# megaease/easevoice-trainer

Hardware: AMD Instinct MI355X
Metric: audio-seconds/sec trained (s2) (higher is better)
Workload: dtype bf16; 1 GPU; s2 SoVITS generator+discriminator GAN step, batch=16/GPU, 4 s 32 kHz clips (T=200 frames), configs/s2.json, random-init weights; global_batch=16, parallelism=dp1, launch=hip-graph replay (3 graphs/step)

## Files before the change

easevoice_trainer_amd/csrc/conv1d.hip:

```cpp
#include "evt_common.h"
#include "../../include/evt.h"
#include "conv_p.h"
#include "wgrad_epi.h"

extern "C" int evt_grouped_supported(const evt_conv1d_params* c);
extern "C" int evt_grouped_fwd(const evt_conv1d_params* c, const void* x, const void* w_reg, const float* bias, void* y,
                               void* stream);
extern "C" int evt_grouped_bwd_data(const evt_conv1d_params* c, const void* dy, const void* y, const void* w_reg,
                                    void* dx, void* stream);
extern "C" int evt_grouped_bwd_data_add(const evt_conv1d_params* c, const void* dy, const void* y, const void* w_reg,
                                        const void* dx_add, void* dx, void* stream);
extern "C" int evt_grouped_bwd_weight(const evt_conv1d_params* c, const void* x, const void* dy, const void* y,
                                      float* dw, void* stream);

extern "C" int evt_small_kind(const evt_conv1d_params* c);
extern "C" int evt_cout1_fwd(const evt_conv1d_params* c, const void* x, const void* w_reg, const float* bias, void* y,
                             void* stream);
extern "C" int evt_cout1_bwd_weight(const evt_conv1d_params* c, const void* x, const void* dy, const void* y, float* dw,
                                    float* dbias, float* ws, long ws_floats, void* stream);
extern "C" int evt_cin1_bwd_weight(const evt_conv1d_params* c, const void* x, const void* dy, const void* y, float* dw,
                                   float* dbias, float* ws, long ws_floats, void* stream);
extern "C" int evt_cin1_fwd(const evt_conv1d_params* c, const void* x, const void* w_reg, const float* bias, void* y,
                            void* stream);
extern "C" int evt_cin1_bwd_data(const evt_conv1d_params* c, const void* dy, const void* y, const void* w_reg,
// ... 1107 lines not shown
  const int d1 = c->transposed ? c->cout : c->cin / c->groups;
  o->d0 = d0; o->d1 = d1; o->k = c->k; o->stride = c->stride;
  pick_ck(c->dtype, d1, c->k, 1, &o->reg_ck, &o->reg_nchunk, &o->reg_kp);
  o->reg_elems = (int64_t)d0 * o->reg_nchunk * o->reg_kp * o->reg_ck;
  if (c->stride == 1) {
    pick_ck(c->dtype, d0, c->k, 1, &o->alt_ck, &o->alt_nchunk, &o->alt_kp);
    o->alt_nphase = 1;
  } else {
    const int J = (c->k + c->stride - 1) / c->stride;
    pick_ck(c->dtype, d0, J, 1, &o->alt_ck, &o->alt_nchunk, &o->alt_kp);
    o->alt_nphase = c->stride;
  }
  o->alt_elems = (int64_t)o->alt_nphase * d1 * o->alt_nchunk * o->alt_kp * o->alt_ck;
  return EVT_OK;
}

int evt_conv1d_fwd(const evt_conv1d_params* c, const void* x, const void* w_reg, const void* w_alt,
                   const float* bias, const void* res, void* y, void* stream) {
  int rc = valid(c);
  if (rc) return rc;
  if (!x || !y) return EVT_EINVAL;
  hipStream_t st = (hipStream_t)stream;
  const bool use_igemm = c->impl != EVT_IMPL_NAIVE && igemm_ok(c);
  if (c->impl == EVT_IMPL_IGEMM && !use_igemm) return EVT_ENOTSUP;
  const int lout = evt_conv1d_lout(c);
  evt_wlayout l; evt_conv1d_layout(c, &l);
  if (w_reg && evt_conv::rows16_eligible(c, c->nseq * c->lin, c->cout, c->cin,
                                         res || c->in_slope != 1.f || c->out_act != EVT_ACT_NONE))
    return evt_conv::launch_rows16(x, w_reg, bias, y, c->nseq * c->lin, c->cout, c->cin, st);
  evt_set_last_tag("conv_naive_fwd");
  if (c->impl != EVT_IMPL_NAIVE && !res && evt_grouped_supported(c)) {
    if (!w_reg) return EVT_EINVAL;
    evt_set_last_tag("grouped_fwd");
    return evt_grouped_fwd(c, x, w_reg, bias, y, stream);
  }
  if (c->impl != EVT_IMPL_NAIVE && !res && evt_small_kind(c) == 1) {
    if (!w_reg) return EVT_EINVAL;
    return evt_cout1_fwd(c, x, w_reg, bias, y, stream);
  }
  if (c->impl != EVT_IMPL_NAIVE && !res && evt_small_kind(c) == 2) {
    if (!w_reg) return EVT_EINVAL;
    return evt_cin1_fwd(c, x, w_reg, bias, y, stream);
  }
  if (!use_igemm) {
    if (!w_reg) return EVT_EINVAL;
    NvP p = make_nvp(c);
    p.x = x; p.w = w_reg; p.bias = bias; p.res = res; p.y = y;
    const long total = (long)c->nseq * lout * c->cout;
    const int blocks = (int)((total + 255) / 256 > 65535 * 8 ? 65535 * 8 : (total + 255) / 256);
    if (c->dtype == EVT_DT_HALF) hipLaunchKernelGGL(conv_naive_fwd<h16_t>, dim3(blocks), dim3(256), 0, st, p);
    else hipLaunchKernelGGL(conv_naive_fwd<float>, dim3(blocks), dim3(256), 0, st, p);
    return evt_check_launch();
  }
  const void* w = c->transposed ? w_alt : w_reg;
  if (!w) return EVT_EINVAL;
  ConvP p{};
  p.x = x; p.xact = nullptr; p.w = w; p.bias = bias; p.res = res; p.gate = nullptr; p.y = y;
  p.nseq = c->nseq; p.Lin = c->lin; p.Lout = lout; p.Cin = c->cin; p.Cout = c->cout;
  p.in_slope = c->in_slope; p.xact_kind = 0; p.xact_slope = 1.f; p.out_act = c->out_act; p.out_slope = c->out_slope;
  p.gate_slope = 1.f;
  int nphase = 1;
  if (!c->transposed) {
    p.KHp = l.reg_kp; p.nchunk = l.reg_nchunk;
    p.s_in = c->stride; p.dil = c->dil; p.off_in = -c->pad;
    p.s_out = 1; p.off_out = 0; p.off_out_phase = 0; p.Q = lout; p.w_phase_stride = 0;
  } else {
    p.KHp = l.alt_kp; p.nchunk = l.alt_nchunk; p.dil = 1; p.s_in = 1;
    if (c->stride == 1) {
      p.off_in = c->pad - (c->k - 1); p.s_out = 1; p.off_out = 0; p.off_out_phase = 0; p.Q = lout;
      p.w_phase_stride = 0;
    } else {
      const int J = (c->k + c->stride - 1) / c->stride;
      nphase = c->stride;
      p.off_in = -(J - 1); p.s_out = c->stride; p.off_out = -c->pad; p.off_out_phase = 1;
      p.Q = (lout - 1 + c->pad) / c->stride + 1;
      p.w_phase_stride = (long)c->cout * l.alt_nchunk * l.alt_kp * l.alt_ck;
    }
  }
  return launch_igemm(c->dtype, p, c->cout, c->cin, nphase, st, c->impl == EVT_IMPL_AUTO);
}

int evt_conv1d_bwd_data(const evt_conv1d_params* c, const void* dy, const void* y, const void* w_reg,
                        const void* w_alt, const void* x, const void* dx_add, void* dx, void* stream) {
  int rc = valid(c);
  if (rc) return rc;
  if (!dy || !dx) return EVT_EINVAL;
  if (c->out_act != EVT_ACT_NONE && !y) return EVT_EINVAL;
  if (c->in_slope != 1.f && !x) return EVT_EINVAL;
  hipStream_t st = (hipStream_t)stream;
  const bool use_igemm = c->impl != EVT_IMPL_NAIVE && igemm_ok(c);
  if (c->impl == EVT_IMPL_IGEMM && !use_igemm) return EVT_ENOTSUP;
  const int lout = evt_conv1d_lout(c);
  evt_wlayout l; evt_conv1d_layout(c, &l);
  const void* ysv = c->out_act != EVT_ACT_NONE ? y : nullptr;
  const void* gate = c->in_slope != 1.f ? x : nullptr;
  if (w_alt && evt_conv::rows16_eligible(c, c->nseq * c->lin, c->cin, c->cout, ysv || gate || dx_add))
    return evt_conv::launch_rows16(dy, w_alt, nullptr, dx, c->nseq * c->lin, c->cin, c->cout, st);
  evt_set_last_tag("conv_naive_bwd_data");
  if (c->impl != EVT_IMPL_NAIVE && !gate && evt_grouped_supported(c)) {
    if (!w_reg) return EVT_EINVAL;
    evt_set_last_tag("grouped_bwd_data");
    return evt_grouped_bwd_data_add(c, dy, y, w_reg, dx_add, dx, stream);
  }
  if (c->impl != EVT_IMPL_NAIVE && evt_small_kind(c) != 0) {
    if (!w_reg) return EVT_EINVAL;
    rc = evt_small_kind(c) == 1 ? evt_cout1_bwd_data(c, dy, y, w_reg, gate, dx_add, dx, stream)
                                : evt_cin1_bwd_data(c, dy, y, w_reg, gate, dx_add, dx, stream);
    if (rc != EVT_ENOTSUP) return rc;
  }
  if (!use_igemm) {
    if (!w_reg) return EVT_EINVAL;
    NvP p = make_nvp(c);
    p.x = dy; p.y_in = ysv; p.w = w_reg; p.gate = gate; p.res = dx_add; p.y = dx;
    const long total = (long)c->nseq * c->lin * c->cin;
    const int blocks = (int)((total + 255) / 256 > 65535 * 8 ? 65535 * 8 : (total + 255) / 256);
    if (c->dtype == EVT_DT_HALF) hipLaunchKernelGGL(conv_naive_bwd_data<h16_t>, dim3(blocks), dim3(256), 0, st, p);
    else hipLaunchKernelGGL(conv_naive_bwd_data<float>, dim3(blocks), dim3(256), 0, st, p);
    return evt_check_launch();
  }
  const void* w = c->transposed ? w_reg : w_alt;
  if (!w) return EVT_EINVAL;
  ConvP p{};
  p.x = dy; p.xact = ysv; p.w = w; p.bias = nullptr; p.res = dx_add; p.gate = gate; p.y = dx;
  p.nseq = c->nseq; p.Lin = lout; p.Lout = c->lin; p.Cin = c->cout; p.Cout = c->cin;
  p.in_slope = 1.f; p.xact_kind = c->out_act; p.xact_slope = c->out_slope; p.out_act = EVT_ACT_NONE;
  p.out_slope = 1.f; p.gate_slope = c->in_slope;
  int nphase = 1;
  if (!c->transposed) {
    p.KHp = l.alt_kp; p.nchunk = l.alt_nchunk;
    if (c->stride == 1) {
      p.s_in = 1; p.dil = c->dil; p.off_in = c->pad - (c->k - 1) * c->dil;
      p.s_out = 1; p.off_out = 0; p.off_out_phase = 0; p.Q = c->lin; p.w_phase_stride = 0;
    } else {
      const int J = (c->k + c->stride - 1) / c->stride;
      nphase = c->stride;
      p.s_in = 1; p.dil = 1; p.off_in = -(J - 1);
      p.s_out = c->stride; p.off_out = -c->pad; p.off_out_phase = 1;
      p.Q = (c->lin - 1 + c->pad) / c->stride + 1;
      p.w_phase_stride = (long)c->cin * l.alt_nchunk * l.alt_kp * l.alt_ck;
    }
  } else {
    p.KHp = l.reg_kp; p.nchunk = l.reg_nchunk;
    p.s_in = c->stride; p.dil = 1; p.off_in = -c->pad;
    p.s_out = 1; p.off_out = 0; p.off_out_phase = 0; p.Q = c->lin; p.w_phase_stride = 0;
  }
  return launch_igemm(c->dtype, p, c->cin, c->cout, nphase, st, c->impl == EVT_IMPL_AUTO);
}

int evt_conv1d_bwd_weight(const evt_conv1d_params* c, const void* x, const void* dy, const void* y, float* dw,
                          float* dbias, void* stream) {
  return evt_conv1d_bwd_weight_parts(c, x, dy, y, dw, dbias, nullptr, stream);
}

int evt_conv1d_bwd_weight_parts(const evt_conv1d_params* c, const void* x, const void* dy, const void* y, float* dw,
                                float* dbias, evt_wgrad_parts* sp, void* stream) {
  int rc = valid(c);
  if (rc) return rc;
  if (!x || !dy || !dw) return EVT_EINVAL;
  int used_host = 0;
  if (sp) {
    sp->used = 0;
    if (sp->parts < 1 || !sp->used_dev || sp->prev_used < 0 || sp->prev_used > sp->parts) return EVT_EINVAL;
    if (sp->parts > 1 && (!sp->dw_extra || sp->part_stride <= 0)) return EVT_EINVAL;
    if (sp->ws && sp->ws_floats <= 0) return EVT_EINVAL;
  }
  if (c->out_act != EVT_ACT_NONE && !y) return EVT_EINVAL;
  hipStream_t st = (hipStream_t)stream;
  const int lout = evt_conv1d_lout(c);
  const void* ysv = c->out_act != EVT_ACT_NONE ? y : nullptr;
  evt_wlayout l; evt_conv1d_layout(c, &l);
  const bool grouped = c->impl != EVT_IMPL_NAIVE && evt_grouped_supported(c);
  const bool igemm_path = !grouped && c->impl != EVT_IMPL_NAIVE && igemm_ok(c) && l.reg_kp <= 64;
  WgP p{};
  p.dw = dw; p.nseq = c->nseq; p.KH = c->k; p.KHp = l.reg_kp; p.s = c->stride; p.dil = c->dil; p.off = -c->pad;
  if (!c->transposed) {
    p.A = dy; p.Aact = ysv; p.aact_kind = c->out_act; p.aact_slope = c->out_slope; p.a_slope = 1.f;
    p.B = x; p.Bact = nullptr; p.bact_kind = 0; p.bact_slope = 1.f; p.b_slope = c->in_slope;
    p.LA = lout; p.CA = c->cout; p.LB = c->lin; p.CB = c->cin; p.Q = lout;
  } else {
    p.A = x; p.Aact = nullptr; p.aact_kind = 0; p.aact_slope = 1.f; p.a_slope = c->in_slope;
    p.B = dy; p.Bact = ysv; p.bact_kind = c->out_act; p.bact_slope = c->out_slope; p.b_slope = 1.f;
    p.LA = c->lin; p.CA = c->cin; p.LB = lout; p.CB = c->cout; p.Q = c->lin;
  }
  p.dbias = nullptr;
  if (sp) {
    p.dw_extra = sp->dw_extra; p.part_stride = sp->part_stride; p.parts = sp->parts; p.prev_used = sp->prev_used;
    p.db_part = sp->db_part; p.used = sp->used_dev; p.used_host = &used_host; p.dirty0 = sp->dirty0 || sp->prev_used > 0;
  }
  const bool gemm_w = igemm_path && c->impl == EVT_IMPL_AUTO && !c->transposed && evt_conv::wgrad_gemm_eligible(p, c->dtype);
  const bool halo_w = !gemm_w && igemm_path && c->impl == EVT_IMPL_AUTO && evt_conv::wgrad_halo_eligible(p, c->dtype);
  const bool deep_w = !gemm_w && !halo_w && igemm_path && c->impl == EVT_IMPL_AUTO && evt_conv::wgrad_deep_eligible(p, c->dtype);
  const bool ring_w = !deep_w && !halo_w && igemm_path && c->impl == EVT_IMPL_AUTO && evt_conv::wgrad_ring_eligible(p, c->dtype);
  const bool cin1 = !grouped && c->impl != EVT_IMPL_NAIVE && evt_small_kind(c) == 2;
  const bool cout1 = !grouped && c->impl != EVT_IMPL_NAIVE && evt_small_kind(c) == 1;
  const bool fuse_bias = dbias && ((igemm_path && c->dtype == EVT_DT_HALF && !c->transposed) || cin1 || cout1);
  float* ws = sp ? sp->ws : nullptr;
  const long ws_floats = sp ? (long)sp->ws_floats : 0;
  if (dbias && !fuse_bias) {
    const long rows = (long)c->nseq * lout;
    const int V = c->dtype == EVT_DT_HALF ? 8 : 4;
    int blocks;
    float* wsb = nullptr;
    if (c->cout % V == 0 && c->cout / V <= 256) {
      long rpb = (rows + 255) / 256;
      if (rpb < 16) rpb = 16;
      blocks = (int)((rows + rpb - 1) / rpb);
      if (ws && blocks >= 2 && (long)blocks * c->cout <= ws_floats) wsb = ws;
      if (c->dtype == EVT_DT_HALF)
        hipLaunchKernelGGL(colsum_act2<h16_t>, dim3(blocks), dim3(256), 0, st, (const h16_t*)dy, (const h16_t*)ysv,
                           dbias, rows, c->cout, c->out_act, c->out_slope, (int)rpb, wsb);
      else
        hipLaunchKernelGGL(colsum_act2<float>, dim3(blocks), dim3(256), 0, st, (const float*)dy, (const float*)ysv,
                           dbias, rows, c->cout, c->out_act, c->out_slope, (int)rpb, wsb);
    } else {
      const int rpb = 64;
      blocks = (int)((rows + rpb - 1) / rpb);
      if (ws && blocks >= 2 && (long)blocks * c->cout <= ws_floats) wsb = ws;
      if (c->dtype == EVT_DT_HALF)
        hipLaunchKernelGGL(colsum_act<h16_t>, dim3(blocks), dim3(256), 0, st, (const h16_t*)dy, (const h16_t*)ysv,
                           dbias, rows, c->cout, c->out_act, c->out_slope, rpb, wsb);
      else
        hipLaunchKernelGGL(colsum_act<float>, dim3(blocks), dim3(256), 0, st, (const float*)dy, (const float*)ysv,
                           dbias, rows, c->cout, c->out_act, c->out_slope, rpb, wsb);
    }
    rc = evt_check_launch();
    if (rc) return rc;
    if (wsb) {
      rc = evt_conv::launch_fold_partials(wsb, c->cout, blocks, dbias, c->cout, st);
      if (rc) return rc;
    }
  }
  evt_set_last_tag("conv_naive_bwd_weight");
  if (grouped) {
    evt_set_last_tag("grouped_bwd_weight");
    return evt_grouped_bwd_weight(c, x, dy, y, dw, stream);
  }
  if (cout1) return evt_cout1_bwd_weight(c, x, dy, y, dw, dbias, ws, ws_floats, stream);
  if (cin1) return evt_cin1_bwd_weight(c, x, dy, y, dw, dbias, ws, ws_floats, stream);
  const bool use_igemm = igemm_path;
  if (c->impl == EVT_IMPL_IGEMM && !use_igemm) return EVT_ENOTSUP;
  if (!use_igemm) {
    NvP p = make_nvp(c);
    p.x = x; p.res = dy; p.y_in = ysv; p.dw = dw;
    const int d1n = c->transposed ? c->cout : c->cin / c->groups;
    const int d0n = c->transposed ? c->cin : c->cout;
    const long elems = (long)d0n * d1n * c->k;
    const long pos = (long)c->nseq * (c->transposed ? c->lin : lout);
    long split = (4096 + elems - 1) / elems;
    const long maxsplit = (pos + 2047) / 2048;
    if (split > maxsplit) split = maxsplit;
    if (split < 1) split = 1;
    p.nsplit = (int)split;
    if (c->dtype == EVT_DT_HALF)
      hipLaunchKernelGGL(conv_naive_bwd_weight<h16_t>, dim3((unsigned)elems, p.nsplit), dim3(256), 0, st, p);
    else
      hipLaunchKernelGGL(conv_naive_bwd_weight<float>, dim3((unsigned)elems, p.nsplit), dim3(256), 0, st, p);
    return evt_check_launch();
  }
  if (gemm_w) {
    p.dbias = fuse_bias ? dbias : nullptr;
    p.parts = 0;
    return evt_conv::launch_wgrad_gemm(p, st);
  }
  if (halo_w || deep_w || ring_w) {
    p.dbias = fuse_bias ? dbias : nullptr;
    if (!p.dbias) p.db_part = nullptr;
    rc = halo_w ? evt_conv::launch_wgrad_halo(p, st) : (deep_w ? evt_conv::launch_wgrad_deep(p, st) : evt_conv::launch_wgrad_ring(p, st));
    if (sp) sp->used = used_host;
    return rc;
  }
  if (c->dtype == EVT_DT_HALF) {
    p.dbias = fuse_bias ? dbias : nullptr;
    p.ws = ws; p.ws_floats = ws_floats;
    if (p.parts < 2) p.parts = 0;
    rc = launch_wgrad_tr(p, st);
    if (sp && rc != EVT_ENOTSUP) sp->used = used_host;
    if (rc != EVT_ENOTSUP) return rc;
    p.parts = 0;
    if (fuse_bias) {
      const long rows = (long)c->nseq * lout;
      hipLaunchKernelGGL(colsum_act<h16_t>, dim3((int)((rows + 63) / 64)), dim3(256), 0, st, (const h16_t*)dy,
                         (const h16_t*)ysv, dbias, rows, c->cout, c->out_act, c->out_slope, 64, (float*)nullptr);
      rc = evt_check_launch();
      if (rc) return rc;
    }
  }
  p.dbias = nullptr;
  return launch_wgrad(c->dtype, p, st);
}

}
```

easevoice_trainer_amd/csrc/conv_deep.hip:

```cpp
#include "conv_p.h"
#include "wgrad_epi.h"

namespace evt_conv {
namespace {

__device__ __attribute__((aligned(256))) unsigned int g_zero_page[64];

typedef __attribute__((address_space(1))) const void* gptr_t;
typedef __attribute__((address_space(3))) void* lptr_t;

__device__ __forceinline__ void glds16(const void* g, void* l) {
  __builtin_amdgcn_global_load_lds((gptr_t)g, (lptr_t)l, 16, 0, 0);
}

constexpr int BM = 128, BN = 128, BK = 64;

template <int TM, int TN, int MI, int NJ>
__device__ __forceinline__ void store_tile_staged(const ConvP& p, unsigned char* smem, const f32x4 (&acc)[MI][NJ], int wr,
                                                  int wc, int n, int g, int yi, int pb, int phase, int total_units) {
  constexpr int PITCH = TM * 2 + 16;
  constexpr int CPR = TM / 8;
  constexpr int RPP = 256 / CPR;
  f32x4 bv[MI];
#pragma unroll
// ... 380 lines not shown
          "=&v"(bh[3]), "=&v"(bh[4])
        : "v"(aa[0]), "v"(aa[1]), "v"(aa[2]), "v"(aa[3]), "v"(ba)
        : "memory");
  } else {
    asm volatile(
        "ds_read_b64_tr_b16 %0, %18 offset:8192\n\t"
        "ds_read_b64_tr_b16 %4, %18 offset:9216\n\t"
        "ds_read_b64_tr_b16 %1, %19 offset:8192\n\t"
        "ds_read_b64_tr_b16 %5, %19 offset:9216\n\t"
        "ds_read_b64_tr_b16 %2, %20 offset:8192\n\t"
        "ds_read_b64_tr_b16 %6, %20 offset:9216\n\t"
        "ds_read_b64_tr_b16 %3, %21 offset:8192\n\t"
        "ds_read_b64_tr_b16 %7, %21 offset:9216\n\t"
        "ds_read_b64_tr_b16 %8, %22 offset:2048\n\t"
        "ds_read_b64_tr_b16 %13, %22 offset:2304\n\t"
        "ds_read_b64_tr_b16 %9, %22 offset:6144\n\t"
        "ds_read_b64_tr_b16 %14, %22 offset:6400\n\t"
        "ds_read_b64_tr_b16 %10, %22 offset:10240\n\t"
        "ds_read_b64_tr_b16 %15, %22 offset:10496\n\t"
        "ds_read_b64_tr_b16 %11, %22 offset:14336\n\t"
        "ds_read_b64_tr_b16 %16, %22 offset:14592\n\t"
        "ds_read_b64_tr_b16 %12, %22 offset:18432\n\t"
        "ds_read_b64_tr_b16 %17, %22 offset:18688\n\t"
        "s_waitcnt lgkmcnt(0)\n\t"
        : "=&v"(al[0]), "=&v"(al[1]), "=&v"(al[2]), "=&v"(al[3]), "=&v"(ah[0]), "=&v"(ah[1]), "=&v"(ah[2]), "=&v"(ah[3]),
          "=&v"(bl[0]), "=&v"(bl[1]), "=&v"(bl[2]), "=&v"(bl[3]), "=&v"(bl[4]), "=&v"(bh[0]), "=&v"(bh[1]), "=&v"(bh[2]),
          "=&v"(bh[3]), "=&v"(bh[4])
        : "v"(aa[0]), "v"(aa[1]), "v"(aa[2]), "v"(aa[3]), "v"(ba)
        : "memory");
  }
  union { uint4 u; h16x8 v; } r;
#pragma unroll
  for (int i = 0; i < 4; ++i) { r.u = make_uint4(al[i].x, al[i].y, ah[i].x, ah[i].y); a[i] = r.v; }
#pragma unroll
  for (int t = 0; t < WKT; ++t) { r.u = make_uint4(bl[t].x, bl[t].y, bh[t].x, bh[t].y); b[t] = r.v; }
}

__global__ __launch_bounds__(256, 2) void wgrad_deep(WgP p, int stages_per_split) {
  extern __shared__ __attribute__((aligned(1024))) unsigned char smem[];
  const int tid = threadIdx.x, lane = tid & 63;
  const int wave = __builtin_amdgcn_readfirstlane(tid >> 6);
  const int j16 = lane & 15, g8 = lane >> 4;
  const int wr = wave >> 1, wc = wave & 1;

  int bx = blockIdx.x;
  int ch, tgi, atile;
  if (p.xcd_order) {
    const int xcd = bx & 7, j = bx >> 3;
    const int na = (p.CA >> 7) >> 1, nc = p.nchunk >> 2;
    const int cl = j % nc, r = j / nc;
    tgi = r % p.ntapgrp;
    const int al = r / p.ntapgrp;
    atile = (xcd & 1) * na + al;
    ch = (xcd >> 1) * nc + cl;
  } else {
    ch = bx % p.nchunk; bx /= p.nchunk;
    tgi = bx % p.ntapgrp;
    atile = bx / p.ntapgrp;
  }
  const int t0 = tgi * WKT;
  const int ntap = min(WKT, p.KHp - t0);
  const int a0 = atile * 128;

  const h16_t* Ag = reinterpret_cast<const h16_t*>(p.A);
  const h16_t* Bg = reinterpret_cast<const h16_t*>(p.B);
  const int total_units = p.nseq * p.Q;
  const int nstages = (total_units + WPOS - 1) / WPOS;
  const int st_begin = blockIdx.y * stages_per_split;
  const int st_end = min(nstages, st_begin + stages_per_split);
  if (st_begin >= st_end) return;

  const h16_t* zsrc = reinterpret_cast<const h16_t*>(g_zero_page);
  int arow[4], acol[4];
#pragma unroll
  for (int i = 0; i < 4; ++i) {
    arow[i] = wave * 16 + i * 4 + (lane >> 4);
    const int f = 2 * ((arow[i] & 3) | (((arow[i] >> 3) & 1) << 2));
    acol[i] = a0 + (((lane & 15) ^ f) * 8);
  }
  const int brow = wave * 16 + (lane >> 2);
  const int bcol = ch * 32 + (((lane & 3) ^ (2 * ((brow >> 3) & 1))) * 8);

  auto issue = [&](int st, int buf) {
    unsigned char* base = smem + buf * WSTAGE;
    const int u0 = st * WPOS;
#pragma unroll
    for (int i = 0; i < 4; ++i) {
      const int u = u0 + arow[i];
      const h16_t* src = u < total_units ? Ag + (long)u * p.CA + acol[i] : zsrc;
      glds16(src, base + wave * 4096 + i * 1024);
    }
    const int u = u0 + brow;
    const bool uok = u < total_units;
    const int seq = uok ? u / p.Q : 0;
    const int q = u - seq * p.Q;
    const int r0 = q * p.s + t0 * p.dil + p.off;
    const h16_t* rsrc = Bg + ((long)seq * p.LB + r0) * p.CB + bcol;
#pragma unroll
    for (int t = 0; t < WKT; ++t) {
      const int r = r0 + t * p.dil;
      const bool ok = uok && (unsigned)r < (unsigned)p.LB;
      const h16_t* src = ok ? rsrc + (long)t * p.dil * p.CB : zsrc;
      glds16(src, base + WA_BYTES + t * WB_BYTES + wave * 1024);
    }
  };

  f32x4 acc[4][WKT];
#pragma unroll
  for (int i = 0; i < 4; ++i)
#pragma unroll
    for (int t = 0; t < WKT; ++t) acc[i][t] = f32x4{0.f, 0.f, 0.f, 0.f};
  const bool do_bias = p.dbias != nullptr && ch == 0 && tgi == 0;
  f32x4 bacc[4];
#pragma unroll
  for (int i = 0; i < 4; ++i) bacc[i] = f32x4{0.f, 0.f, 0.f, 0.f};

  const unsigned lds0 = (unsigned)(uintptr_t)smem;
  const int frow = g8 * 8 + (j16 >> 2);
  const int fa = 2 * ((frow & 3) | (((frow >> 3) & 1) << 2));
  const int fb = 2 * ((frow >> 3) & 1);
  const int half = (j16 & 1) * 8;
  int a_off[4];
#pragma unroll
  for (int i = 0; i < 4; ++i) a_off[i] = frow * 256 + (((wr * 8 + i * 2 + ((j16 & 3) >> 1)) ^ fa) * 16) + half;
  const int b_off = WA_BYTES + frow * 64 + (((wc * 2 + ((j16 & 3) >> 1)) ^ fb) * 16) + half;

  issue(st_begin, 0);
  for (int st = st_begin; st < st_end; ++st) {
    const int buf = (st - st_begin) & 1;
    __syncthreads();
    if (st + 1 < st_end) issue(st + 1, buf ^ 1);
    const unsigned sbase = lds0 + buf * WSTAGE;
    unsigned aa[4];
#pragma unroll
    for (int i = 0; i < 4; ++i) aa[i] = sbase + a_off[i];
    const unsigned ba = sbase + b_off;
    h16x8 a[4], b[WKT];
    tr_load_step<0>(aa, ba, a, b);
#pragma unroll
    for (int t = 0; t < WKT; ++t)
      if (t < ntap)
#pragma unroll
        for (int i = 0; i < 4; ++i) acc[i][t] = EVT_MFMA_16x16x32(a[i], b[t], acc[i][t], 0, 0, 0);
    if (do_bias) wg_bias_mma<4>(bacc, a, wc);
    tr_load_step<1>(aa, ba, a, b);
#pragma unroll
    for (int t = 0; t < WKT; ++t)
      if (t < ntap)
#pragma unroll
        for (int i = 0; i < 4; ++i) acc[i][t] = EVT_MFMA_16x16x32(a[i], b[t], acc[i][t], 0, 0, 0);
    if (do_bias) wg_bias_mma<4>(bacc, a, wc);
  }
  if (do_bias) wg_finish_bias_mma<4>(p, bacc, a0, wr, wc, g8, j16, blockIdx.y);
  wg_finish<4, WKT>(p, smem, acc, ntap, a0, ch, t0, wr, wc, g8, j16, blockIdx.y);
}

constexpr int GKT = 4;
constexpr int GSTAGE = WA_BYTES + GKT * WB_BYTES;

template <int KS>
__device__ __forceinline__ void tr_load_step_g(const unsigned (&aa)[4], unsigned ba, h16x8 (&a)[4], h16x8 (&b)[GKT]) {
  uint2 al[4], ah[4], bl[GKT], bh[GKT];
  if constexpr (KS == 0) {
    asm volatile(
        "ds_read_b64_tr_b16 %0, %16 offset:0\n\t"
        "ds_read_b64_tr_b16 %4, %16 offset:1024\n\t"
        "ds_read_b64_tr_b16 %1, %17 offset:0\n\t"
        "ds_read_b64_tr_b16 %5, %17 offset:1024\n\t"
        "ds_read_b64_tr_b16 %2, %18 offset:0\n\t"
        "ds_read_b64_tr_b16 %6, %18 offset:1024\n\t"
        "ds_read_b64_tr_b16 %3, %19 offset:0\n\t"
        "ds_read_b64_tr_b16 %7, %19 offset:1024\n\t"
        "ds_read_b64_tr_b16 %8, %20 offset:0\n\t"
        "ds_read_b64_tr_b16 %12, %20 offset:256\n\t"
        "ds_read_b64_tr_b16 %9, %20 offset:4096\n\t"
        "ds_read_b64_tr_b16 %13, %20 offset:4352\n\t"
        "ds_read_b64_tr_b16 %10, %20 offset:8192\n\t"
        "ds_read_b64_tr_b16 %14, %20 offset:8448\n\t"
        "ds_read_b64_tr_b16 %11, %20 offset:12288\n\t"
        "ds_read_b64_tr_b16 %15, %20 offset:12544\n\t"
        "s_waitcnt lgkmcnt(0)\n\t"
        : "=&v"(al[0]), "=&v"(al[1]), "=&v"(al[2]), "=&v"(al[3]), "=&v"(ah[0]), "=&v"(ah[1]), "=&v"(ah[2]), "=&v"(ah[3]),
          "=&v"(bl[0]), "=&v"(bl[1]), "=&v"(bl[2]), "=&v"(bl[3]), "=&v"(bh[0]), "=&v"(bh[1]), "=&v"(bh[2]), "=&v"(bh[3])
        : "v"(aa[0]), "v"(aa[1]), "v"(aa[2]), "v"(aa[3]), "v"(ba)
        : "memory");
  } else {
    asm volatile(
        "ds_read_b64_tr_b16 %0, %16 offset:8192\n\t"
        "ds_read_b64_tr_b16 %4, %16 offset:9216\n\t"
        "ds_read_b64_tr_b16 %1, %17 offset:8192\n\t"
        "ds_read_b64_tr_b16 %5, %17 offset:9216\n\t"
        "ds_read_b64_tr_b16 %2, %18 offset:8192\n\t"
        "ds_read_b64_tr_b16 %6, %18 offset:9216\n\t"
        "ds_read_b64_tr_b16 %3, %19 offset:8192\n\t"
        "ds_read_b64_tr_b16 %7, %19 offset:9216\n\t"
        "ds_read_b64_tr_b16 %8, %20 offset:2048\n\t"
        "ds_read_b64_tr_b16 %12, %20 offset:2304\n\t"
        "ds_read_b64_tr_b16 %9, %20 offset:6144\n\t"
        "ds_read_b64_tr_b16 %13, %20 offset:6400\n\t"
        "ds_read_b64_tr_b16 %10, %20 offset:10240\n\t"
        "ds_read_b64_tr_b16 %14, %20 offset:10496\n\t"
        "ds_read_b64_tr_b16 %11, %20 offset:14336\n\t"
        "ds_read_b64_tr_b16 %15, %20 offset:14592\n\t"
        "s_waitcnt lgkmcnt(0)\n\t"
        : "=&v"(al[0]), "=&v"(al[1]), "=&v"(al[2]), "=&v"(al[3]), "=&v"(ah[0]), "=&v"(ah[1]), "=&v"(ah[2]), "=&v"(ah[3]),
          "=&v"(bl[0]), "=&v"(bl[1]), "=&v"(bl[2]), "=&v"(bl[3]), "=&v"(bh[0]), "=&v"(bh[1]), "=&v"(bh[2]), "=&v"(bh[3])
        : "v"(aa[0]), "v"(aa[1]), "v"(aa[2]), "v"(aa[3]), "v"(ba)
        : "memory");
  }
  union { uint4 u; h16x8 v; } r;
#pragma unroll
  for (int i = 0; i < 4; ++i) { r.u = make_uint4(al[i].x, al[i].y, ah[i].x, ah[i].y); a[i] = r.v; }
#pragma unroll
  for (int t = 0; t < GKT; ++t) { r.u = make_uint4(bl[t].x, bl[t].y, bh[t].x, bh[t].y); b[t] = r.v; }
}

template <int NS>
__global__ __launch_bounds__(256, NS > 2 ? 1 : 2) void wgrad_gemm(WgP p, int stages_per_split) {
  extern __shared__ __attribute__((aligned(1024))) unsigned char smem[];
  const int tid = threadIdx.x, lane = tid & 63;
  const int wave = __builtin_amdgcn_readfirstlane(tid >> 6);
  const int j16 = lane & 15, g8 = lane >> 4;
  const int wr = wave >> 1, wc = wave & 1;

  int tile = blockIdx.x, split = blockIdx.y;
  if (p.xcd_order) {
    const int lin = blockIdx.y * gridDim.x + blockIdx.x;
    const int xcd = lin & 7, idx = lin >> 3;
    tile = idx % (int)gridDim.x;
    split = xcd + 8 * (idx / (int)gridDim.x);
  }
  const int ngrp = p.nchunk / GKT;
  const int cg = tile % ngrp;
  const int atile = tile / ngrp;
  const int a0 = atile * 128;

  const h16_t* Ag = reinterpret_cast<const h16_t*>(p.A);
  const h16_t* Bg = reinterpret_cast<const h16_t*>(p.B);
  const int total_units = p.nseq * p.Q;
  const int nstages = (total_units + WPOS - 1) / WPOS;
  const int st_begin = split * stages_per_split;
  const int st_end = min(nstages, st_begin + stages_per_split);
  if (st_begin >= st_end) return;

  const h16_t* zsrc = reinterpret_cast<const h16_t*>(g_zero_page);
  int arow[4], acol[4];
#pragma unroll
  for (int i = 0; i < 4; ++i) {
    arow[i] = wave * 16 + i * 4 + (lane >> 4);
    const int f = 2 * ((arow[i] & 3) | (((arow[i] >> 3) & 1) << 2));
    acol[i] = a0 + (((lane & 15) ^ f) * 8);
  }
  const int brow = wave * 16 + (lane >> 2);
  const int bcol = cg * 128 + (((lane & 3) ^ (2 * ((brow >> 3) & 1))) * 8);

  auto issue = [&](int st, int buf) {
    unsigned char* base = smem + buf * GSTAGE;
    const int u0 = st * WPOS;
#pragma unroll
    for (int i = 0; i < 4; ++i) {
      const int u = u0 + arow[i];
      const h16_t* src = u < total_units ? Ag + (long)u * p.CA + acol[i] : zsrc;
      glds16(src, base + wave * 4096 + i * 1024);
    }
    const int u = u0 + brow;
    const bool uok = u < total_units;
    const h16_t* rsrc = Bg + (long)(uok ? u : 0) * p.CB + bcol;
#pragma unroll
    for (int t = 0; t < GKT; ++t) glds16(uok ? rsrc + t * 32 : zsrc, base + WA_BYTES + t * WB_BYTES + wave * 1024);
  };

  f32x4 acc[4][GKT];
#pragma unroll
  for (int i = 0; i < 4; ++i)
#pragma unroll
    for (int t = 0; t < GKT; ++t) acc[i][t] = f32x4{0.f, 0.f, 0.f, 0.f};
  const int bgrp = ngrp < 4 ? ngrp : 4;
  const bool do_bias = p.dbias != nullptr && cg < bgrp && wc == 0;
  bool mine[4];
#pragma unroll
  for (int i = 0; i < 4; ++i) mine[i] = do_bias && (i % bgrp) == cg;
  h16x8 ones;
#pragma unroll
  for (int e = 0; e < 8; ++e) ones[e] = (evt_hn)1.0f;
  f32x4 bacc[4];
#pragma unroll
  for (int i = 0; i < 4; ++i) bacc[i] = f32x4{0.f, 0.f, 0.f, 0.f};

  const unsigned lds0 = (unsigned)(uintptr_t)smem;
  const int frow = g8 * 8 + (j16 >> 2);
  const int fa = 2 * ((frow & 3) | (((frow >> 3) & 1) << 2));
  const int fb = 2 * ((frow >> 3) & 1);
  const int half = (j16 & 1) * 8;
  int a_off[4];
#pragma unroll
  for (int i = 0; i < 4; ++i) a_off[i] = frow * 256 + (((wr * 8 + i * 2 + ((j16 & 3) >> 1)) ^ fa) * 16) + half;
  const int b_off = WA_BYTES + frow * 64 + (((wc * 2 + ((j16 & 3) >> 1)) ^ fb) * 16) + half;

  const int nst = st_end - st_begin;
  constexpr int G = 4 + GKT;
#pragma unroll
  for (int s = 0; s < NS - 1; ++s)
    if (s < nst) issue(st_begin + s, s);
  for (int st = st_begin; st < st_end; ++st) {
    const int s = st - st_begin;
    const int buf = s % NS;
    wait_groups<G, NS - 2>(min(NS - 2, nst - 1 - s));
// ... 189 lines not shown
        "ds_read_b64_tr_b16 %5, %11 offset:1024\n\t"
        "ds_read_b64_tr_b16 %2, %12 offset:0\n\t"
        "ds_read_b64_tr_b16 %6, %12 offset:1024\n\t"
        "ds_read_b64_tr_b16 %3, %13 offset:0\n\t"
        "ds_read_b64_tr_b16 %7, %13 offset:1024\n\t"
        "ds_read_b64_tr_b16 %8, %14 offset:0\n\t"
        "ds_read_b64_tr_b16 %9, %14 offset:256\n\t"
        "s_waitcnt lgkmcnt(0)\n\t"
        : "=&v"(al[0]), "=&v"(al[1]), "=&v"(al[2]), "=&v"(al[3]), "=&v"(ah[0]), "=&v"(ah[1]), "=&v"(ah[2]), "=&v"(ah[3]), "=&v"(bl[0]), "=&v"(bh[0])
        : "v"(aa[0]), "v"(aa[1]), "v"(aa[2]), "v"(aa[3]), "v"(ba)
        : "memory");
    } else {
    asm volatile(
        "ds_read_b64_tr_b16 %0, %10 offset:8192\n\t"
        "ds_read_b64_tr_b16 %4, %10 offset:9216\n\t"
        "ds_read_b64_tr_b16 %1, %11 offset:8192\n\t"
        "ds_read_b64_tr_b16 %5, %11 offset:9216\n\t"
        "ds_read_b64_tr_b16 %2, %12 offset:8192\n\t"
        "ds_read_b64_tr_b16 %6, %12 offset:9216\n\t"
        "ds_read_b64_tr_b16 %3, %13 offset:8192\n\t"
        "ds_read_b64_tr_b16 %7, %13 offset:9216\n\t"
        "ds_read_b64_tr_b16 %8, %14 offset:2048\n\t"
        "ds_read_b64_tr_b16 %9, %14 offset:2304\n\t"
        "s_waitcnt lgkmcnt(0)\n\t"
        : "=&v"(al[0]), "=&v"(al[1]), "=&v"(al[2]), "=&v"(al[3]), "=&v"(ah[0]), "=&v"(ah[1]), "=&v"(ah[2]), "=&v"(ah[3]), "=&v"(bl[0]), "=&v"(bh[0])
        : "v"(aa[0]), "v"(aa[1]), "v"(aa[2]), "v"(aa[3]), "v"(ba)
        : "memory");
    }
    union { uint4 u; h16x8 v; } r;
#pragma unroll
    for (int i = 0; i < 4; ++i) { r.u = make_uint4(al[i].x, al[i].y, ah[i].x, ah[i].y); a[i] = r.v; }
#pragma unroll
    for (int t = 0; t < 1; ++t) { r.u = make_uint4(bl[t].x, bl[t].y, bh[t].x, bh[t].y); b[t] = r.v; }
  }
};
template <> struct TrStep<4, 3> {
  template <int KS>
  static __device__ __forceinline__ void load(const unsigned (&aa)[4], unsigned ba, h16x8 (&a)[4], h16x8 (&b)[3]) {
    uint2 al[4], ah[4], bl[3], bh[3];
    if constexpr (KS == 0) {
    asm volatile(
        "ds_read_b64_tr_b16 %0, %14 offset:0\n\t"
        "ds_read_b64_tr_b16 %4, %14 offset:1024\n\t"
        "ds_read_b64_tr_b16 %1, %15 offset:0\n\t"
        "ds_read_b64_tr_b16 %5, %15 offset:1024\n\t"
        "ds_read_b64_tr_b16 %2, %16 offset:0\n\t"
        "ds_read_b64_tr_b16 %6, %16 offset:1024\n\t"
        "ds_read_b64_tr_b16 %3, %17 offset:0\n\t"
        "ds_read_b64_tr_b16 %7, %17 offset:1024\n\t"
        "ds_read_b64_tr_b16 %8, %18 offset:0\n\t"
        "ds_read_b64_tr_b16 %11, %18 offset:256\n\t"
        "ds_read_b64_tr_b16 %9, %18 offset:4096\n\t"
        "ds_read_b64_tr_b16 %12, %18 offset:4352\n\t"
        "ds_read_b64_tr_b16 %10, %18 offset:8192\n\t"
        "ds_read_b64_tr_b16 %13, %18 offset:8448\n\t"
        "s_waitcnt lgkmcnt(0)\n\t"
        : "=&v"(al[0]), "=&v"(al[1]), "=&v"(al[2]), "=&v"(al[3]), "=&v"(ah[0]), "=&v"(ah[1]), "=&v"(ah[2]), "=&v"(ah[3]), "=&v"(bl[0]), "=&v"(bl[1]), "=&v"(bl[2]), "=&v"(bh[0]), "=&v"(bh[1]), "=&v"(bh[2])
        : "v"(aa[0]), "v"(aa[1]), "v"(aa[2]), "v"(aa[3]), "v"(ba)
        : "memory");
    } else {
    asm volatile(
        "ds_read_b64_tr_b16 %0, %14 offset:8192\n\t"
        "ds_read_b64_tr_b16 %4, %14 offset:9216\n\t"
        "ds_read_b64_tr_b16 %1, %15 offset:8192\n\t"
        "ds_read_b64_tr_b16 %5, %15 offset:9216\n\t"
        "ds_read_b64_tr_b16 %2, %16 offset:8192\n\t"
        "ds_read_b64_tr_b16 %6, %16 offset:9216\n\t"
        "ds_read_b64_tr_b16 %3, %17 offset:8192\n\t"
        "ds_read_b64_tr_b16 %7, %17 offset:9216\n\t"
        "ds_read_b64_tr_b16 %8, %18 offset:2048\n\t"
        "ds_read_b64_tr_b16 %11, %18 offset:2304\n\t"
        "ds_read_b64_tr_b16 %9, %18 offset:6144\n\t"
        "ds_read_b64_tr_b16 %12, %18 offset:6400\n\t"
        "ds_read_b64_tr_b16 %10, %18 offset:10240\n\t"
        "ds_read_b64_tr_b16 %13, %18 offset:10496\n\t"
        "s_waitcnt lgkmcnt(0)\n\t"
        : "=&v"(al[0]), "=&v"(al[1]), "=&v"(al[2]), "=&v"(al[3]), "=&v"(ah[0]), "=&v"(ah[1]), "=&v"(ah[2]), "=&v"(ah[3]), "=&v"(bl[0]), "=&v"(bl[1]), "=&v"(bl[2]), "=&v"(bh[0]), "=&v"(bh[1]), "=&v"(bh[2])
        : "v"(aa[0]), "v"(aa[1]), "v"(aa[2]), "v"(aa[3]), "v"(ba)
        : "memory");
    }
    union { uint4 u; h16x8 v; } r;
#pragma unroll
    for (int i = 0; i < 4; ++i) { r.u = make_uint4(al[i].x, al[i].y, ah[i].x, ah[i].y); a[i] = r.v; }
#pragma unroll
    for (int t = 0; t < 3; ++t) { r.u = make_uint4(bl[t].x, bl[t].y, bh[t].x, bh[t].y); b[t] = r.v; }
  }
};
template <> struct TrStep<4, 5> {
  template <int KS>
  static __device__ __forceinline__ void load(const unsigned (&aa)[4], unsigned ba, h16x8 (&a)[4], h16x8 (&b)[5]) {
    uint2 al[4], ah[4], bl[5], bh[5];
    if constexpr (KS == 0) {
    asm volatile(
        "ds_read_b64_tr_b16 %0, %18 offset:0\n\t"
        "ds_read_b64_tr_b16 %4, %18 offset:1024\n\t"
        "ds_read_b64_tr_b16 %1, %19 offset:0\n\t"
        "ds_read_b64_tr_b16 %5, %19 offset:1024\n\t"
        "ds_read_b64_tr_b16 %2, %20 offset:0\n\t"
        "ds_read_b64_tr_b16 %6, %20 offset:1024\n\t"
        "ds_read_b64_tr_b16 %3, %21 offset:0\n\t"
        "ds_read_b64_tr_b16 %7, %21 offset:1024\n\t"
        "ds_read_b64_tr_b16 %8, %22 offset:0\n\t"
        "ds_read_b64_tr_b16 %13, %22 offset:256\n\t"
        "ds_read_b64_tr_b16 %9, %22 offset:4096\n\t"
        "ds_read_b64_tr_b16 %14, %22 offset:4352\n\t"
        "ds_read_b64_tr_b16 %10, %22 offset:8192\n\t"
        "ds_read_b64_tr_b16 %15, %22 offset:8448\n\t"
        "ds_read_b64_tr_b16 %11, %22 offset:12288\n\t"
        "ds_read_b64_tr_b16 %16, %22 offset:12544\n\t"
        "ds_read_b64_tr_b16 %12, %22 offset:16384\n\t"
        "ds_read_b64_tr_b16 %17, %22 offset:16640\n\t"
        "s_waitcnt lgkmcnt(0)\n\t"
        : "=&v"(al[0]), "=&v"(al[1]), "=&v"(al[2]), "=&v"(al[3]), "=&v"(ah[0]), "=&v"(ah[1]), "=&v"(ah[2]), "=&v"(ah[3]), "=&v"(bl[0]), "=&v"(bl[1]), "=&v"(bl[2]), "=&v"(bl[3]), "=&v"(bl[4]), "=&v"(bh[0]), "=&v"(bh[1]), "=&v"(bh[2]), "=&v"(bh[3]), "=&v"(bh[4])
        : "v"(aa[0]), "v"(aa[1]), "v"(aa[2]), "v"(aa[3]), "v"(ba)
        : "memory");
    } else {
    asm volatile(
        "ds_read_b64_tr_b16 %0, %18 offset:8192\n\t"
        "ds_read_b64_tr_b16 %4, %18 offset:9216\n\t"
        "ds_read_b64_tr_b16 %1, %19 offset:8192\n\t"
        "ds_read_b64_tr_b16 %5, %19 offset:9216\n\t"
        "ds_read_b64_tr_b16 %2, %20 offset:8192\n\t"
        "ds_read_b64_tr_b16 %6, %20 offset:9216\n\t"
        "ds_read_b64_tr_b16 %3, %21 offset:8192\n\t"
        "ds_read_b64_tr_b16 %7, %21 offset:9216\n\t"
        "ds_read_b64_tr_b16 %8, %22 offset:2048\n\t"
        "ds_read_b64_tr_b16 %13, %22 offset:2304\n\t"
        "ds_read_b64_tr_b16 %9, %22 offset:6144\n\t"
        "ds_read_b64_tr_b16 %14, %22 offset:6400\n\t"
        "ds_read_b64_tr_b16 %10, %22 offset:10240\n\t"
        "ds_read_b64_tr_b16 %15, %22 offset:10496\n\t"
        "ds_read_b64_tr_b16 %11, %22 offset:14336\n\t"
        "ds_read_b64_tr_b16 %16, %22 offset:14592\n\t"
        "ds_read_b64_tr_b16 %12, %22 offset:18432\n\t"
        "ds_read_b64_tr_b16 %17, %22 offset:18688\n\t"
        "s_waitcnt lgkmcnt(0)\n\t"
        : "=&v"(al[0]), "=&v"(al[1]), "=&v"(al[2]), "=&v"(al[3]), "=&v"(ah[0]), "=&v"(ah[1]), "=&v"(ah[2]), "=&v"(ah[3]), "=&v"(bl[0]), "=&v"(bl[1]), "=&v"(bl[2]), "=&v"(bl[3]), "=&v"(bl[4]), "=&v"(bh[0]), "=&v"(bh[1]), "=&v"(bh[2]), "=&v"(bh[3]), "=&v"(bh[4])
        : "v"(aa[0]), "v"(aa[1]), "v"(aa[2]), "v"(aa[3]), "v"(ba)
        : "memory");
    }
    union { uint4 u; h16x8 v; } r;
#pragma unroll
    for (int i = 0; i < 4; ++i) { r.u = make_uint4(al[i].x, al[i].y, ah[i].x, ah[i].y); a[i] = r.v; }
#pragma unroll
    for (int t = 0; t < 5; ++t) { r.u = make_uint4(bl[t].x, bl[t].y, bh[t].x, bh[t].y); b[t] = r.v; }
  }
};

template <int MA> __device__ __forceinline__ int a_swz(int row) {
  return MA == 4 ? 2 * ((row & 3) | (((row >> 3) & 1) << 2)) : 2 * (((row >> 1) & 1) | (((row >> 3) & 1) << 1));
}

template <int MA, int KT, int NS>
__global__ __launch_bounds__(256) void wgrad_ring(WgP p, int stages_per_split) {
  constexpr int AROW = 64 * MA;
  constexpr int ABYTES = WPOS * AROW;
  constexpr int STAGE = ABYTES + KT * WB_BYTES;
  constexpr int G = MA + KT;
  constexpr int RPI = 16 / MA;
  extern __shared__ __attribute__((aligned(1024))) unsigned char smem[];
  const int tid = threadIdx.x, lane = tid & 63;
  const int wave = __builtin_amdgcn_readfirstlane(tid >> 6);
  const int j16 = lane & 15, g8 = lane >> 4;
  const int wr = wave >> 1, wc = wave & 1;

  int bx = blockIdx.x;
  const int split = blockIdx.y;
  const int ch = bx % p.nchunk; bx /= p.nchunk;
  const int tgi = bx % p.ntapgrp;
  const int atile = bx / p.ntapgrp;
  const int t0 = tgi * KT;
  const int ntap = min(KT, p.KHp - t0);
  const int a0 = atile * 32 * MA;

  const h16_t* Ag = reinterpret_cast<const h16_t*>(p.A);
  const h16_t* Bg = reinterpret_cast<const h16_t*>(p.B);
  const int total_units = p.nseq * p.Q;
  const int nstages = (total_units + WPOS - 1) / WPOS;
  const int st_begin = split * stages_per_split;
  const int nst = min(nstages, st_begin + stages_per_split) - st_begin;
  if (nst <= 0) return;

  const h16_t* zsrc = reinterpret_cast<const h16_t*>(g_zero_page);
  int arow[MA], acol[MA];
#pragma unroll
  for (int i = 0; i < MA; ++i) {
    arow[i] = wave * 16 + i * RPI + lane / (4 * MA);
    acol[i] = a0 + (((lane % (4 * MA)) ^ a_swz<MA>(arow[i])) * 8);
  }
  const int brow = wave * 16 + (lane >> 2);
  const int bcol = ch * 32 + (((lane & 3) ^ (2 * ((brow >> 3) & 1))) * 8);

  auto issue = [&](int s) {
    unsigned char* base = smem + (s % NS) * STAGE;
    const int u0 = (st_begin + s) * WPOS;
#pragma unroll
    for (int i = 0; i < MA; ++i) {
      const int u = u0 + arow[i];
      glds16(u < total_units ? Ag + (long)u * p.CA + acol[i] : zsrc, base + wave * (16 * AROW) + i * 1024);
    }
    const int u = u0 + brow;
    const bool uok = u < total_units;
    const int seq = uok ? u / p.Q : 0;
    const int q = u - seq * p.Q;
    const int r0 = q * p.s + t0 * p.dil + p.off;
    const h16_t* rsrc = Bg + ((long)seq * p.LB + r0) * p.CB + bcol;
#pragma unroll
    for (int t = 0; t < KT; ++t) {
      const int r = r0 + t * p.dil;
      const bool ok = uok && (unsigned)r < (unsigned)p.LB;
      glds16(ok ? rsrc + (long)t * p.dil * p.CB : zsrc, base + ABYTES + t * WB_BYTES + wave * 1024);
    }
  };

  f32x4 acc[MA][KT];
#pragma unroll
  for (int i = 0; i < MA; ++i)
#pragma unroll
    for (int t = 0; t < KT; ++t) acc[i][t] = f32x4{0.f, 0.f, 0.f, 0.f};
  const bool do_bias = p.dbias != nullptr && ch == 0 && tgi == 0;
  f32x4 bacc[MA];
#pragma unroll
  for (int i = 0; i < MA; ++i) bacc[i] = f32x4{0.f, 0.f, 0.f, 0.f};

  const unsigned lds0 = (unsigned)(uintptr_t)smem;
  const int frow = g8 * 8 + (j16 >> 2);
  const int fa = a_swz<MA>(frow);
  const int fb = 2 * ((frow >> 3) & 1);
  const int half = (j16 & 1) * 8;
  int a_off[MA];
#pragma unroll
  for (int i = 0; i < MA; ++i) a_off[i] = frow * AROW + (((wr * 2 * MA + i * 2 + ((j16 & 3) >> 1)) ^ fa) * 16) + half;
  const int b_off = ABYTES + frow * 64 + (((wc * 2 + ((j16 & 3) >> 1)) ^ fb) * 16) + half;

#pragma unroll
  for (int s = 0; s < NS - 1; ++s)
    if (s < nst) issue(s);
  for (int s = 0; s < nst; ++s) {
    const int ahead = min(NS - 2, nst - 1 - s);
    wait_groups<G, NS - 2>(ahead);
    __builtin_amdgcn_s_barrier();
    asm volatile("" ::: "memory");
    if (s + NS - 1 < nst) issue(s + NS - 1);
    const unsigned sbase = lds0 + (s % NS) * STAGE;
    unsigned aa[MA];
#pragma unroll
    for (int i = 0; i < MA; ++i) aa[i] = sbase + a_off[i];
    const unsigned ba = sbase + b_off;
    h16x8 a[MA], b[KT];
    TrStep<MA, KT>::template load<0>(aa, ba, a, b);
#pragma unroll
    for (int t = 0; t < KT; ++t)
      if (t < ntap)
#pragma unroll
        for (int i = 0; i < MA; ++i) acc[i][t] = EVT_MFMA_16x16x32(a[i], b[t], acc[i][t], 0, 0, 0);
    if (do_bias) wg_bias_mma<MA>(bacc, a, wc);
    TrStep<MA, KT>::template load<1>(aa, ba, a, b);
#pragma unroll
    for (int t = 0; t < KT; ++t)
      if (t < ntap)
#pragma unroll
        for (int i = 0; i < MA; ++i) acc[i][t] = EVT_MFMA_16x16x32(a[i], b[t], acc[i][t], 0, 0, 0);
    if (do_bias) wg_bias_mma<MA>(bacc, a, wc);
    asm volatile("" ::: "memory");
  }
  if (do_bias) wg_finish_bias_mma<MA>(p, bacc, a0, wr, wc, g8, j16, split);
  wg_finish<MA, KT>(p, smem, acc, ntap, a0, ch, t0, wr, wc, g8, j16, split);
}

}

static int deep_kind(const ConvP& p, int dtype, int out_ch, int k_ch, int nphase);

bool deep_eligible(const ConvP& p, int dtype, int out_ch, int k_ch, int nphase) {
  return deep_kind(p, dtype, out_ch, k_ch, nphase) != 0;
}

static int deep_kind(const ConvP& p, int dtype, int out_ch, int k_ch, int nphase) {
  if (dtype != EVT_DT_HALF) return 0;
  if (k_ch % 32 || out_ch % 64) return 0;
  if (p.xact || p.in_slope != 1.f) return 0;
  if (p.nchunk * 32 != k_ch) return 0;
  if ((long)p.nseq * p.Q >= (1L << 31) - BN) return 0;
  const long units = (long)p.nseq * p.Q;
  constexpr long min128 = 192;
  if (out_ch % BM == 0 && ((units + BN - 1) / BN) * (out_ch / BM) * nphase >= min128) return 2;
  if (k_ch % BK == 0 && ((units + 63) / 64) * (out_ch / 64) * nphase >= 32) return 1;
  return 0;
}


int launch_conv_deep(const ConvP& p_in, int out_ch, int k_ch, int nphase, hipStream_t st) {
  ConvP p = p_in;
  const int kind = deep_kind(p, EVT_DT_HALF, out_ch, k_ch, nphase);
  if (kind == 0) return EVT_ENOTSUP;
  if (kind == 1) {
    p.Y = out_ch / 64;
    p.P = (int)(((long)p.nseq * p.Q + 63) / 64);
    p.U = 0;
    constexpr int NS = 4;
    static bool attr1 = false;
    const size_t lds1 = (size_t)NS * (64 + 64) * 128;
    if (!attr1) {
      if (hipFuncSetAttribute(reinterpret_cast<const void*>(&conv_ring<2, 2, NS>),
                              hipFuncAttributeMaxDynamicSharedMemorySize, (int)lds1) != hipSuccess)
        return EVT_ELAUNCH;
      attr1 = true;
    }
    evt_set_last_tag("conv_ring<bf16, 64, 64, 64, x4>");
    hipLaunchKernelGGL((conv_ring<2, 2, NS>), dim3(8 * ((p.P + 7) / 8) * p.Y, nphase), dim3(256), lds1, st, p);
    return evt_check_launch();
  }
  p.Y = out_ch / BM;
  p.P = (int)(((long)p.nseq * p.Q + BN - 1) / BN);
  p.U = 0;
  const bool short_k = (k_ch / 64) * p.KHp <= 12;
  if (k_ch % 64 || short_k) {
    static bool attr32 = false;
    const size_t lds32 = 2 * STAGE32 > 128 * 272 ? 2 * STAGE32 : 128 * 272;
    if (!attr32) {
      if (hipFuncSetAttribute(reinterpret_cast<const void*>(&conv_deep32), hipFuncAttributeMaxDynamicSharedMemorySize,
                              (int)lds32) != hipSuccess)
        return EVT_ELAUNCH;
      attr32 = true;
    }
    evt_set_last_tag("conv_deep32<bf16, 128, 128, 32>");
    hipLaunchKernelGGL(conv_deep32, dim3(8 * ((p.P + 7) / 8) * p.Y, nphase), dim3(256), lds32, st, p);
    return evt_check_launch();
  }
  static bool attr = false;
  const size_t lds = 2 * STAGE_BYTES;
  if (!attr) {
    if (hipFuncSetAttribute(reinterpret_cast<const void*>(&conv_deep), hipFuncAttributeMaxDynamicSharedMemorySize,
                            (int)lds) != hipSuccess)
      return EVT_ELAUNCH;
    attr = true;
  }
  const int gx = 8 * ((p.P + 7) / 8) * p.Y;
  evt_set_last_tag("conv_deep<bf16, 128, 128, 64>");
  hipLaunchKernelGGL(conv_deep, dim3(gx, nphase), dim3(256), lds, st, p);
  return evt_check_launch();
}

void wgrad_pick_split(const WgP& p, long tiles, int nstages, long target, int min_stages, int* nsplit, int* per) {
  long split = (target + tiles - 1) / tiles;
  if (split > nstages / min_stages) split = nstages / min_stages;
  if (p.parts > 0 && split > p.parts) split = p.parts;
  if (split < 1) split = 1;
  *per = (int)((nstages + split - 1) / split);
  *nsplit = (nstages + *per - 1) / *per;
}

bool wgrad_deep_eligible(const WgP& p, int dtype) {
  if (dtype != EVT_DT_HALF) return false;
  if (p.CA % 128 || p.CB % 32) return false;
  if (p.Aact || p.Bact || p.a_slope != 1.f || p.b_slope != 1.f) return false;
  if (p.LA != p.Q) return false;
  if (p.KHp < 3) return false;
  if ((long)p.nseq * p.Q >= (1L << 31) - WPOS) return false;
  const long tiles = (long)(p.CA / 128) * (p.CB / 32) * ((p.KHp + WKT - 1) / WKT);
  const long nstages = ((long)p.nseq * p.Q + WPOS - 1) / WPOS;
  long split = (1024 + tiles - 1) / tiles;
  if (split > nstages / 8) split = nstages / 8;
  return split >= 1 && tiles * split >= 256;
}

int launch_wgrad_deep(const WgP& p_in, hipStream_t st) {
  WgP p = p_in;
  if (!wgrad_deep_eligible(p, EVT_DT_HALF)) return EVT_ENOTSUP;
  p.nchunk = p.CB / 32;
  p.ntapgrp = (p.KHp + WKT - 1) / WKT;
  const long tiles = (long)(p.CA / 128) * p.nchunk * p.ntapgrp;
  p.xcd_order = ((p.CA / 128) % 2 == 0 && p.nchunk % 4 == 0) ? 1 : 0;
  const int nstages = (int)(((long)p.nseq * p.Q + WPOS - 1) / WPOS);
  int nsplit, per;
  wgrad_pick_split(p, tiles, nstages, p.parts > 0 ? 512 : 1024, 8, &nsplit, &per);
  p.nsplit = nsplit;
  p.now_used = p.prev_used > nsplit ? p.prev_used : nsplit;
  if (p.parts > 0 && p.used_host) *p.used_host = p.now_used;
  static bool attr = false;
  const size_t lds = 2 * WSTAGE;
  if (!attr) {
    if (hipFuncSetAttribute(reinterpret_cast<const void*>(&wgrad_deep), hipFuncAttributeMaxDynamicSharedMemorySize,
                            (int)lds) != hipSuccess)
      return EVT_ELAUNCH;
    attr = true;
  }
  evt_set_last_tag("wgrad_deep<bf16, 128, 5x32, 64>");
  hipLaunchKernelGGL(wgrad_deep, dim3((unsigned)tiles, p.nsplit), dim3(256), lds, st, p, per);
  return evt_check_launch();
}

bool wgrad_gemm_eligible(const WgP& p, int dtype) {
  if (dtype != EVT_DT_HALF) return false;
  if (p.KH != 1 || p.KHp != 1 || p.s != 1 || p.off != 0) return false;
  if (p.CA % 128 || p.CB % 128) return false;
  if (p.Aact || p.Bact || p.a_slope != 1.f || p.b_slope != 1.f) return false;
  if (p.LA != p.Q || p.LB != p.Q) return false;
  const long units = (long)p.nseq * p.Q;
  if (units >= (1L << 31) - WPOS) return false;
  return units >= 2048;
}

static int launch_wgrad_gemm_grid(const WgP& p, long tiles, int per, hipStream_t st);

int launch_wgrad_gemm(const WgP& p_in, hipStream_t st) {
  WgP p = p_in;
  if (!wgrad_gemm_eligible(p, EVT_DT_HALF)) return EVT_ENOTSUP;
  p.nchunk = p.CB / 32;
  p.ntapgrp = 1;
  const long tiles = (long)(p.CA / 128) * (p.CB / 128);
  const int nstages = (int)(((long)p.nseq * p.Q + WPOS - 1) / WPOS);
  constexpr long target = 256;
  long split = (target + tiles - 1) / tiles;
  if (split > nstages / 8) split = nstages / 8;
  if (split < 1) split = 1;
  const int per = (int)((nstages + split - 1) / split);
  split = (nstages + per - 1) / per;
  p.xcd_order = 0;
  if (nstages >= 64) {
    const long s8 = (split + 7) / 8 * 8;
    const int per8 = (int)((nstages + s8 - 1) / s8);
    if ((long)per8 * (s8 - 1) < nstages) {
      split = s8;
      p.xcd_order = 1;
      p.nsplit = (int)split;
      return launch_wgrad_gemm_grid(p, tiles, per8, st);
    }
  }
  p.nsplit = (int)split;
  return launch_wgrad_gemm_grid(p, tiles, per, st);
}

template <int NS>
static int launch_wgrad_gemm_ns(const WgP& p, long tiles, int per, hipStream_t st) {
  static bool attr = false;
  const size_t lds = NS * GSTAGE;
  if (!attr) {
    if (hipFuncSetAttribute(reinterpret_cast<const void*>(&wgrad_gemm<NS>), hipFuncAttributeMaxDynamicSharedMemorySize,
                            (int)lds) != hipSuccess)
      return EVT_ELAUNCH;
    attr = true;
  }
  evt_set_last_tag("wgrad_gemm<bf16, 128, 128, 64, x%d>", NS);
  hipLaunchKernelGGL(wgrad_gemm<NS>, dim3((unsigned)tiles, p.nsplit), dim3(256), lds, st, p, per);
  return evt_check_launch();
}

static int launch_wgrad_gemm_grid(const WgP& p, long tiles, int per, hipStream_t st) {
  return launch_wgrad_gemm_ns<2>(p, tiles, per, st);
}

template <int MA, int KT, int NS>
static int launch_ring_inst(const WgP& p, int per, hipStream_t st) {
  constexpr size_t lds = (size_t)NS * (WPOS * 64 * MA + KT * WB_BYTES);
  static bool attr = false;
  if (!attr) {
    if (hipFuncSetAttribute(reinterpret_cast<const void*>(&wgrad_ring<MA, KT, NS>),
                            hipFuncAttributeMaxDynamicSharedMemorySize, (int)lds) != hipSuccess)
      return EVT_ELAUNCH;
    attr = true;
  }
  const long tiles = (long)(p.CA / (32 * MA)) * p.nchunk * p.ntapgrp;
  evt_set_last_tag("wgrad_ring<bf16, %d, %dx32, 64, x%d>", 32 * MA, KT, NS);
  hipLaunchKernelGGL((wgrad_ring<MA, KT, NS>), dim3((unsigned)tiles, p.nsplit), dim3(256), lds, st, p, per);
  return evt_check_launch();
}

bool wgrad_ring_eligible(const WgP& p, int dtype) {
  if (dtype != EVT_DT_HALF) return false;
  if (p.CA % 64 || p.CB % 32) return false;
  if (p.Aact || p.Bact || p.a_slope != 1.f || p.b_slope != 1.f) return false;
  if (p.LA != p.Q) return false;
  const long units = (long)p.nseq * p.Q;
  if (units >= (1L << 31) - WPOS || units < 512) return false;
  return true;
}

int launch_wgrad_ring(const WgP& p_in, hipStream_t st) {
  WgP p = p_in;
  if (!wgrad_ring_eligible(p, EVT_DT_HALF)) return EVT_ENOTSUP;
  const int KT = p.KHp <= 1 ? 1 : (p.KHp <= 3 ? 3 : 5);
  p.nchunk = p.CB / 32;
  p.ntapgrp = (p.KHp + KT - 1) / KT;
  const int nstages = (int)(((long)p.nseq * p.Q + WPOS - 1) / WPOS);
  const long tiles128 = p.CA % 128 == 0 ? (long)(p.CA / 128) * p.nchunk * p.ntapgrp : 0;
  const int MA = (tiles128 >= 128 || (tiles128 > 0 && tiles128 * (nstages / 4) >= 512)) ? 4 : 2;
  const long tiles = (long)(p.CA / (32 * MA)) * p.nchunk * p.ntapgrp;
  constexpr long target = 256;
  int nsplit, per;
  wgrad_pick_split(p, tiles, nstages, target, 3, &nsplit, &per);
  p.nsplit = nsplit;
  p.now_used = p.prev_used > nsplit ? p.prev_used : nsplit;
  if (p.parts > 0 && p.used_host) *p.used_host = p.now_used;
#define RING(MA_, KT_) (MA_ == 4 && KT_ == 5 ? launch_ring_inst<MA_, KT_, 3>(p, per, st) : launch_ring_inst<MA_, KT_, 4>(p, per, st))
  if (MA == 4) return KT == 1 ? RING(4, 1) : (KT == 3 ? RING(4, 3) : RING(4, 5));
  return KT == 1 ? RING(2, 1) : (KT == 3 ? RING(2, 3) : RING(2, 5));
#undef RING
}

}
```

easevoice_trainer_amd/csrc/conv_p.h:

```cpp
#pragma once
#include "evt_common.h"
#include "../../include/evt.h"
#include <cstdlib>

namespace evt_conv {

struct ConvP {
  const void* x;
  const void* xact;
  const void* w;
  const float* bias;
  const void* res;
  const void* gate;
  void* y;
  int nseq, Lin, Lout, Cin, Cout;
  int KHp;
  int s_in, dil, off_in;
  int s_out, off_out, off_out_phase;
  int Q, U;
  int nchunk;
  long w_phase_stride;
  float in_slope;
  int xact_kind;
  float xact_slope;
  int out_act;
  float out_slope;
  float gate_slope;
  int P, Y;
};

struct WgP {
  const void* A;
  const void* Aact;
  const void* B;
  const void* Bact;
  float* dw;
  int nseq, LA, LB, CA, CB;
  int KH, KHp, s, dil, off, Q;
  int nchunk;
  float a_slope, b_slope;
  int aact_kind, bact_kind;
  float aact_slope, bact_slope;
  int nsplit;
  int ntapgrp;
  int xcd_order;
  float* dbias;
  float* dw_extra;
  long part_stride;
  int parts;
  int prev_used;
  int now_used;
  int dirty0;
  float* db_part;
  int* used;
  int* used_host;
  float* ws;
  long ws_floats;
};

bool deep_eligible(const ConvP& p, int dtype, int out_ch, int k_ch, int nphase);
int launch_conv_deep(const ConvP& p, int out_ch, int k_ch, int nphase, hipStream_t st);
bool narrow_eligible(const ConvP& p, int dtype, int out_ch, int k_ch, int nphase);
int launch_conv_narrow(const ConvP& p, int out_ch, int k_ch, int nphase, hipStream_t st);
bool wgrad_deep_eligible(const WgP& p, int dtype);
int launch_wgrad_deep(const WgP& p, hipStream_t st);
bool wgrad_gemm_eligible(const WgP& p, int dtype);
int launch_wgrad_gemm(const WgP& p, hipStream_t st);
bool wgrad_ring_eligible(const WgP& p, int dtype);
int launch_wgrad_ring(const WgP& p, hipStream_t st);
bool wgrad_halo_eligible(const WgP& p, int dtype);
int launch_wgrad_halo(const WgP& p, hipStream_t st);
int launch_fold_partials(const float* part, long stride, int nb, float* out, long n, hipStream_t st);
int launch_fold_partials2(const float* part, long stride, int nb, float* out, long n, float* out2, long n2, hipStream_t st);
void wgrad_pick_split(const WgP& p, long tiles, int nstages, long target, int min_stages, int* nsplit, int* per);

bool rows16_eligible(const struct evt_conv1d_params* c, int rows, int n_out, int k_red, bool fused);
int launch_rows16(const void* x, const void* w, const float* bias, void* y, int M, int N, int K, hipStream_t st);

}
```

easevoice_trainer_amd/csrc/wgrad_epi.h:

```cpp
#pragma once
#include "conv_p.h"

namespace evt_conv {

__device__ __forceinline__ float* wg_slab(const WgP& p, int s) {
  return s == 0 ? p.dw : p.dw_extra + (long)(s - 1) * p.part_stride;
}

template <int MI, int NT>
__device__ __forceinline__ void wg_store_slab(const WgP& p, float* slab, bool add, float* scratch,
                                              const f32x4 (&acc)[MI][NT], int ntap, int a0, int ch, int t0, int wr, int wc,
                                              int g8, int j16) {
  constexpr int PITCH = NT * 32 + 4;
  constexpr int CPR = NT * 8;
  const int tid = threadIdx.x;
  if constexpr (NT == 1) {
#pragma unroll
    for (int i = 0; i < MI; ++i)
#pragma unroll
      for (int r = 0; r < 4; ++r) {
        const int a = a0 + wr * 16 * MI + i * 16 + g8 * 4 + r;
        float* dst = slab + (((long)a * p.nchunk + ch) * p.KHp + t0) * 32 + wc * 16 + j16;
        *dst = add ? *dst + acc[i][0][r] : acc[i][0][r];
      }
    return;
  }
#pragma unroll
  for (int i = 0; i < MI; ++i) {
    __syncthreads();
#pragma unroll
    for (int t = 0; t < NT; ++t)
#pragma unroll
      for (int r = 0; r < 4; ++r) scratch[(wr * 16 + g8 * 4 + r) * PITCH + t * 32 + wc * 16 + j16] = acc[i][t][r];
    __syncthreads();
    for (int c = tid; c < 32 * CPR; c += 256) {
      const int lr = c / CPR, cc = c - lr * CPR;
      if (cc >= ntap * 8) continue;
      const int a = a0 + (lr >> 4) * 16 * MI + i * 16 + (lr & 15);
      float* dst = slab + (((long)a * p.nchunk + ch) * p.KHp + t0) * 32 + cc * 4;
      f32x4 v = *reinterpret_cast<const f32x4*>(scratch + lr * PITCH + cc * 4);
      if (add) {
        const f32x4 o = *reinterpret_cast<const f32x4*>(dst);
        v += o;
      }
      *reinterpret_cast<f32x4*>(dst) = v;
    }
  }
}

template <int MI, int NT>
__device__ __forceinline__ void wg_finish(const WgP& p, unsigned char* smem, const f32x4 (&acc)[MI][NT], int ntap, int a0,
                                          int ch, int t0, int wr, int wc, int g8, int j16, int split) {
  if (p.parts > 0) {
    if (blockIdx.x == 0 && blockIdx.y == 0 && threadIdx.x == 0) p.used[0] = p.now_used;
    wg_store_slab<MI, NT>(p, wg_slab(p, split), split == 0 ? p.dirty0 != 0 : split < p.prev_used, reinterpret_cast<float*>(smem), acc, ntap,
                          a0, ch, t0, wr, wc, g8, j16);
    return;
  }
#pragma unroll
  for (int t = 0; t < NT; ++t) {
    if (t >= ntap) continue;
#pragma unroll
    for (int i = 0; i < MI; ++i)
#pragma unroll
      for (int r = 0; r < 4; ++r) {
        const int a = a0 + wr * 16 * MI + i * 16 + g8 * 4 + r;
        const long off = (((long)a * p.nchunk + ch) * p.KHp + t0 + t) * 32 + wc * 16 + j16;
        atomicAdd(p.dw + off, acc[i][t][r]);
      }
  }
}

template <int MI>
__device__ __forceinline__ void wg_bias_mma(f32x4 (&bacc)[MI], const h16x8 (&a)[MI], int wc) {
  h16x8 ones;
#pragma unroll
  for (int e = 0; e < 8; ++e) ones[e] = (evt_hn)1.0f;
#pragma unroll
  for (int i = 0; i < MI; ++i)
    if ((i & 1) == wc) bacc[i] = EVT_MFMA_16x16x32(a[i], ones, bacc[i], 0, 0, 0);
}

__device__ __forceinline__ void wg_finish_bias(const WgP& p, int channel, float bsum, int split);

template <int MI>
__device__ __forceinline__ void wg_finish_bias_mma(const WgP& p, const f32x4 (&bacc)[MI], int a0, int wr, int wc, int g8,
                                                   int j16, int split) {
  if (j16 != 0) return;
#pragma unroll
  for (int i = 0; i < MI; ++i)
    if ((i & 1) == wc)
#pragma unroll
      for (int r = 0; r < 4; ++r) wg_finish_bias(p, a0 + wr * 16 * MI + i * 16 + g8 * 4 + r, bacc[i][r], split);
}

__device__ __forceinline__ void wg_finish_bias(const WgP& p, int channel, float bsum, int split) {
  if (p.parts > 0 && p.db_part) {
    float* d = p.db_part + (long)split * p.CA + channel;
    *d = split < p.prev_used ? *d + bsum : bsum;
    if (channel == 0 && split == 0) p.used[1] = p.now_used;
  } else {
    atomicAdd(p.dbias + channel, bsum);
  }
}

}
```

easevoice_trainer_amd/csrc/wgrad_halo.hip:

```cpp
#include "conv_p.h"
#include "wgrad_epi.h"
#include <cstdlib>
#include <type_traits>

namespace evt_conv {
namespace {

__device__ __attribute__((aligned(256))) unsigned int g_zero_page_h[64];

typedef __attribute__((address_space(1))) const void* gptr_t;
typedef __attribute__((address_space(3))) void* lptr_t;

__device__ __forceinline__ void glds16(const void* g, void* l) {
  __builtin_amdgcn_global_load_lds((gptr_t)g, (lptr_t)l, 16, 0, 0);
}

template <int N> __device__ __forceinline__ void wait_vmcnt() { asm volatile("s_waitcnt vmcnt(%0)" ::"n"(N) : "memory"); }
template <int G, int MAXA>
__device__ __forceinline__ void wait_groups(int ahead) {
  if constexpr (MAXA <= 0) { wait_vmcnt<0>(); }
  else {
    if (ahead >= MAXA) wait_vmcnt<(MAXA * G > 63 ? 63 : MAXA * G)>();
    else wait_groups<G, MAXA - 1>(ahead);
  }
// ... 16 lines not shown
template <int MA> __device__ __forceinline__ int a_swz(int row) {
  return MA == 4 ? 2 * ((row & 3) | (((row >> 3) & 1) << 2))
                 : (MA == 2 ? 2 * (((row >> 1) & 1) | (((row >> 3) & 1) << 1)) : 2 * ((row >> 3) & 1));
}

constexpr int HPOS = 64;
constexpr int HROWS = 128;
constexpr int HWIN = HROWS * 64;

template <int MA, int NT, int NS>
__global__ __launch_bounds__(256) void wgrad_halo(WgP p, int spq, int stages_per_split) {
  constexpr int AROW = 64 * MA;
  constexpr int ABYTES = HPOS * AROW;
  constexpr int STAGE = ABYTES + HWIN;
  constexpr int G = MA + 2;
  constexpr int RPI = 16 / MA;
  extern __shared__ __attribute__((aligned(1024))) unsigned char smem[];
  const int tid = threadIdx.x, lane = tid & 63;
  const int wave = __builtin_amdgcn_readfirstlane(tid >> 6);
  const int j16 = lane & 15, g8 = lane >> 4;
  const int wr = wave >> 1, wc = wave & 1;

  const int ch = blockIdx.x % p.nchunk;
  const int a0 = (blockIdx.x / p.nchunk) * 32 * MA;

  const h16_t* Ag = reinterpret_cast<const h16_t*>(p.A);
  const h16_t* Bg = reinterpret_cast<const h16_t*>(p.B);
  const int nstages = p.nseq * spq;
  const int st_begin = blockIdx.y * stages_per_split;
  const int nst = min(nstages, st_begin + stages_per_split) - st_begin;
  if (nst <= 0) return;
  const int hrows = HPOS + (NT - 1) * p.dil;

  const h16_t* zsrc = reinterpret_cast<const h16_t*>(g_zero_page_h);
  int arow[MA], acol[MA];
#pragma unroll
  for (int i = 0; i < MA; ++i) {
    arow[i] = wave * 16 + i * RPI + lane / (4 * MA);
    acol[i] = a0 + (((lane % (4 * MA)) ^ a_swz<MA>(arow[i])) * 8);
  }
  const int brow = wave * 16 + (lane >> 2);
  const int bcol = ch * 32 + (((lane & 3) ^ (2 * ((brow >> 3) & 1))) * 8);

  auto issue = [&](int s) {
    unsigned char* base = smem + (s % NS) * STAGE;
    const int gs = st_begin + s;
    const int seq = gs / spq;
    const int q0 = (gs - seq * spq) * HPOS;
#pragma unroll
    for (int i = 0; i < MA; ++i) {
      const int q = q0 + arow[i];
      glds16(q < p.Q ? Ag + ((long)seq * p.LA + q) * p.CA + acol[i] : zsrc, base + wave * (16 * AROW) + i * 1024);
    }
    const h16_t* rsrc = Bg + ((long)seq * p.LB + q0 + p.off) * p.CB + bcol;
#pragma unroll
    for (int ps = 0; ps < 2; ++ps) {
      const int j = ps * 64 + brow;
      const int r = q0 + p.off + j;
      const bool ok = j < hrows && (unsigned)r < (unsigned)p.LB;
      glds16(ok ? rsrc + (long)j * p.CB : zsrc, base + ABYTES + ps * 4096 + wave * 1024);
    }
  };

  f32x4 acc[MA][NT];
#pragma unroll
  for (int i = 0; i < MA; ++i)
#pragma unroll
    for (int t = 0; t < NT; ++t) acc[i][t] = f32x4{0.f, 0.f, 0.f, 0.f};
  const bool do_bias = p.dbias != nullptr && ch == 0;
  f32x4 bacc[MA];
#pragma unroll
  for (int i = 0; i < MA; ++i) bacc[i] = f32x4{0.f, 0.f, 0.f, 0.f};

  const unsigned lds0 = (unsigned)(uintptr_t)smem;
  const int frow = g8 * 8 + (j16 >> 2);
  const int fa = a_swz<MA>(frow);
  const int half = (j16 & 1) * 8;
  const int cs = (j16 & 3) >> 1;
  int a_off[MA];
#pragma unroll
  for (int i = 0; i < MA; ++i) a_off[i] = frow * AROW + (((wr * 2 * MA + i * 2 + cs) ^ fa) * 16) + half;
  int b_lo[NT], b_hi[NT];
#pragma unroll
  for (int t = 0; t < NT; ++t) {
    const int r0 = frow + t * p.dil, r1 = r0 + 4;
    b_lo[t] = ABYTES + r0 * 64 + (((wc * 2 + cs) ^ (2 * ((r0 >> 3) & 1))) * 16) + half;
    b_hi[t] = ABYTES + r1 * 64 + (((wc * 2 + cs) ^ (2 * ((r1 >> 3) & 1))) * 16) + half;
  }

#pragma unroll
  for (int s = 0; s < NS - 1; ++s)
    if (s < nst) issue(s);
  for (int s = 0; s < nst; ++s) {
    const int ahead = min(NS - 2, nst - 1 - s);
    wait_groups<G, NS - 2>(ahead);
    __builtin_amdgcn_s_barrier();
    asm volatile("" ::: "memory");
    if (s + NS - 1 < nst) issue(s + NS - 1);
    const unsigned sbase = lds0 + (s % NS) * STAGE;
    TrPair fa[2][MA], fb[2][NT];
    auto rd = [&](auto KS, TrPair (&a)[MA], TrPair (&b)[NT]) {
      constexpr int ks = decltype(KS)::value;
#pragma unroll
      for (int i = 0; i < MA; ++i) {
        a[i].lo = tr_rd<ks * 32 * AROW>(sbase + a_off[i]);
        a[i].hi = tr_rd<ks * 32 * AROW + 4 * AROW>(sbase + a_off[i]);
      }
#pragma unroll
      for (int t = 0; t < NT; ++t) {
        b[t].lo = tr_rd<ks * 2048>(sbase + b_lo[t]);
        b[t].hi = tr_rd<ks * 2048>(sbase + b_hi[t]);
      }
    };
    auto landed = [&](TrPair (&a)[MA], TrPair (&b)[NT]) {
#pragma unroll
      for (int i = 0; i < MA; ++i) tr_tie(a[i]);
#pragma unroll
      for (int t = 0; t < NT; ++t) tr_tie(b[t]);
    };
    auto mma = [&](TrPair (&a)[MA], TrPair (&b)[NT]) {
#pragma unroll
      for (int t = 0; t < NT; ++t) {
        const h16x8 bv = tr_join(b[t]);
#pragma unroll
        for (int i = 0; i < MA; ++i) acc[i][t] = EVT_MFMA_16x16x32(tr_join(a[i]), bv, acc[i][t], 0, 0, 0);
      }
      if (do_bias) {
        h16x8 af[MA];
#pragma unroll
        for (int i = 0; i < MA; ++i) af[i] = tr_join(a[i]);
        wg_bias_mma<MA>(bacc, af, wc);
      }
    };
    constexpr bool PIPE = MA * NT * 4 + 2 * (MA + NT) * 4 <= 200;
    rd(std::integral_constant<int, 0>{}, fa[0], fb[0]);
    asm volatile("s_waitcnt lgkmcnt(0)");
    landed(fa[0], fb[0]);
    if constexpr (PIPE) {
      rd(std::integral_constant<int, 1>{}, fa[1], fb[1]);
      mma(fa[0], fb[0]);
      asm volatile("s_waitcnt lgkmcnt(0)");
      landed(fa[1], fb[1]);
      mma(fa[1], fb[1]);
    } else {
      mma(fa[0], fb[0]);
      rd(std::integral_constant<int, 1>{}, fa[0], fb[0]);
      asm volatile("s_waitcnt lgkmcnt(0)");
      landed(fa[0], fb[0]);
      mma(fa[0], fb[0]);
    }
    asm volatile("" ::: "memory");
  }
  if (do_bias) wg_finish_bias_mma<MA>(p, bacc, a0, wr, wc, g8, j16, blockIdx.y);
  wg_finish<MA, NT>(p, smem, acc, NT, a0, ch, 0, wr, wc, g8, j16, blockIdx.y);
}

template <int MA, int NT, int NS>
int launch_inst(const WgP& p, int spq, int per, hipStream_t st) {
  constexpr size_t lds = (size_t)NS * (HPOS * 64 * MA + HWIN);
  static_assert(lds >= 32 * (NT * 32 + 4) * 4, "epilogue scratch");
  static bool attr = false;
  if (!attr) {
    if (hipFuncSetAttribute(reinterpret_cast<const void*>(&wgrad_halo<MA, NT, NS>),
                            hipFuncAttributeMaxDynamicSharedMemorySize, (int)lds) != hipSuccess)
      return EVT_ELAUNCH;
    attr = true;
  }
  const long tiles = (long)(p.CA / (32 * MA)) * p.nchunk;
  evt_set_last_tag("wgrad_halo<bf16, %d, %dx32, 64, x%d>", 32 * MA, NT, NS);
  hipLaunchKernelGGL((wgrad_halo<MA, NT, NS>), dim3((unsigned)tiles, p.nsplit), dim3(256), lds, st, p, spq, per);
  return evt_check_launch();
}

}

bool wgrad_halo_eligible(const WgP& p, int dtype) {
  if (dtype != EVT_DT_HALF) return false;
  if (p.s != 1 || p.KHp != p.KH) return false;
  if (p.KH != 3 && p.KH != 5 && p.KH != 7 && p.KH != 11) return false;
  if ((p.CA % 64 && p.CA != 32) || p.CB % 32) return false;
  if (p.Aact || p.Bact || p.a_slope != 1.f || p.b_slope != 1.f) return false;
  if (p.LA != p.Q) return false;
  if (HPOS + (p.KH - 1) * p.dil > HROWS) return false;
  static const bool all = getenv("EVT_HALO_ALL") != nullptr;
  if (!all && p.CA != 64 && p.CA != 32) return false;
  if (p.CA % 128 == 0 && (long)(p.CA / 128) * (p.CB / 32) >= 128) return false;
  const int spq = (p.Q + HPOS - 1) / HPOS;
  if ((long)spq * HPOS * 10 > (long)p.Q * 13) return false;
  if ((long)p.nseq * spq < 8) return false;
  return true;
}

int launch_wgrad_halo(const WgP& p_in, hipStream_t st) {
  WgP p = p_in;
  if (!wgrad_halo_eligible(p, EVT_DT_HALF)) return EVT_ENOTSUP;
  p.nchunk = p.CB / 32;
  p.ntapgrp = 1;
  const int spq = (p.Q + HPOS - 1) / HPOS;
  const int nstages = p.nseq * spq;
  const long tiles128 = p.CA % 128 == 0 ? (long)(p.CA / 128) * p.nchunk : 0;
  int MA = tiles128 >= 64 ? 4 : 2;
  if (p.CA == 32) MA = 1;
  const long tiles = (long)(p.CA / (32 * MA)) * p.nchunk;
  constexpr long target = 256;
  int nsplit, per;
  wgrad_pick_split(p, tiles, nstages, target, 3, &nsplit, &per);
  p.nsplit = nsplit;
  p.now_used = p.prev_used > nsplit ? p.prev_used : nsplit;
  if (p.parts > 0 && p.used_host) *p.used_host = p.now_used;
#define HALO(MA_, NS_)                                                                                   \
  (p.KH == 3 ? launch_inst<MA_, 3, NS_>(p, spq, per, st)                                                 \
             : p.KH == 5 ? launch_inst<MA_, 5, NS_>(p, spq, per, st)                                     \
                         : p.KH == 7 ? launch_inst<MA_, 7, NS_>(p, spq, per, st) : launch_inst<MA_, 11, NS_>(p, spq, per, st))
  return MA == 4 ? HALO(4, 3) : (MA == 2 ? HALO(2, 4) : HALO(1, 4));
#undef HALO
}

}
```

easevoice_trainer_amd/hip/conv.py:

```python
import ctypes as C
import os
import math

import torch
from torch import nn

from . import lib as L


class ConvSlot:

    __slots__ = ("module", "layout", "reg", "alt", "dw", "bank", "_pcache", "packed_member", "parts", "dw_extra",
                 "db_part", "used", "wg_used", "wg_dirty", "_wgp")

    def __init__(self, module, layout, bank):
        self.module, self.layout, self.bank = module, layout, bank
        self.reg = self.alt = self.dw = None
        self._pcache = {}
        self.packed_member = False
        self.parts, self.dw_extra, self.db_part, self.used, self.wg_used, self._wgp = 1, None, None, None, 0, None
        self.wg_dirty = False

    def params(self, nseq, lin, in_slope, out_act, out_slope):
        key = (nseq, lin, in_slope, out_act, out_slope, self.bank.impl)
# ... 154 lines not shown
            ex_n += (s.parts - 1) * ((s.layout.reg_elems + ALIGN - 1) // ALIGN * ALIGN)
            db_n += s.parts * ((s.layout.d0 + 31) // 32 * 32)
        self._ws = {}
        self.dw_extra_arena = torch.zeros(max(ex_n, 1), dtype=torch.float32, device=device) if self.parts_on else None
        self.db_part_arena = torch.zeros(max(db_n, 1), dtype=torch.float32, device=device) if self.parts_on else None
        for i, (s, (ro, ao)) in enumerate(zip(self.slots, offs)):
            s.reg = self.reg_arena[ro: ro + s.layout.reg_elems]
            s.alt = self.alt_arena[ao: ao + s.layout.alt_elems]
            s.dw = self.dw_arena[ro: ro + s.layout.reg_elems]
            s.used = self.used_all[2 * i: 2 * i + 2]
            if self.parts_on:
                eo, do = ex_offs[i]
                stride = (s.layout.reg_elems + ALIGN - 1) // ALIGN * ALIGN
                s.dw_extra = self.dw_extra_arena[eo: eo + (s.parts - 1) * stride]
                s.db_part = self.db_part_arena[do: do + s.parts * s.layout.d0]
        self._items = self._rows = None
        self._nrows = 0
        self._frags, self._frag_items, self._frag_rows, self._frag_tables = {}, [], [], {}
        self._frag_retired = []

    def build_tables(self):
        items, rows, groups = [], [], []
        self._slot_rows = []
        self._group_of_row = {}
        for i, s in enumerate(self.slots):
            m = s.module
            self._slot_rows.append((len(rows), len(rows) + s.layout.d0))
            v = m.v
            if v.grad is None:
                v.grad = torch.zeros_like(v)
            g = m.weight_g if m.weight_norm else None
            if g is not None and g.grad is None:
                g.grad = torch.zeros_like(g)
            it = L.WPrepItem()
            it.v = v.data_ptr()
            it.g = g.data_ptr() if g is not None else None
            it.reg, it.alt, it.dw = s.reg.data_ptr(), s.alt.data_ptr(), (None if s.packed_member else s.dw.data_ptr())
            it.dv = v.grad.data_ptr()
            it.dg = g.grad.data_ptr() if g is not None else None
            it.lay = s.layout
            it.dtype = self.dt
            it.src_d1 = int(getattr(m, "src_d1", 0))
            if self.parts_on and not s.packed_member:
                it.dw_extra = s.dw_extra.data_ptr() if s.parts > 1 else None
                it.dw_part_stride = (s.layout.reg_elems + 127) // 128 * 128
                it.used = s.used.data_ptr()
                bias = getattr(m, "bias", None)
                if bias is not None and not m.transposed:
                    if bias.grad is None:
                        bias.grad = torch.zeros_like(bias)
                    it.db_part, it.db = s.db_part.data_ptr(), bias.grad.data_ptr()
            items.append(it)
            self._group_of_row[len(rows)] = len(groups)
            rows.extend((i, r) for r in range(s.layout.d0))
            groups.extend((i, r, min(8, s.layout.d0 - r)) for r in range(0, s.layout.d0, 8))
        self._group_of_row[len(rows)] = len(groups)
        self._items = L.struct_to_device(items, self.device)
        self._rows = torch.tensor(rows, dtype=torch.int32, device=self.device).contiguous()
        self._groups = torch.tensor(groups, dtype=torch.int32, device=self.device).contiguous()
        self._nrows = len(rows)
        self._grad_stamp = self._grad_ptrs()

    def _grad_ptrs(self):
        out = []
        for s in self.slots:
            m = s.module
            g = m.weight_g if m.weight_norm else None
            b = getattr(m, "bias", None)
            out.append((m.v.grad.data_ptr() if m.v.grad is not None else 0,
                        g.grad.data_ptr() if (g is not None and g.grad is not None) else 0,
                        b.grad.data_ptr() if (b is not None and b.grad is not None) else 0))
        return out

    def fold(self, lo=None, hi=None):
        if self._items is None:
            self.build_tables()
        lo = 0 if lo is None else lo
        hi = self._nrows if hi is None else hi
        if hi <= lo:
            return
        glo, ghi = self._group_of_row.get(lo), self._group_of_row.get(hi)
        if glo is not None and ghi is not None and os.environ.get("EVT_FOLD_GROUPS", "1") != "0":
            grp = C.c_void_p(self._groups.data_ptr() + 12 * glo)
            L.check(L.lib().evt_wn_fold_groups(L.ptr(self._items), grp, ghi - glo, L.stream_ptr()), "evt_wn_fold_groups")
        else:
            rows = C.c_void_p(self._rows.data_ptr() + 8 * lo)
            L.check(L.lib().evt_wn_fold_multi(L.ptr(self._items), rows, hi - lo, L.stream_ptr()), "evt_wn_fold_multi")
        self._repack_frags(lo, hi)

    def frag(self, slot, which):
        key = (id(slot), which)
        f = self._frags.get(key)
        if f is None:
            lay = slot.layout
            if which == "reg":
                rows, ktot, src, elems = lay.d0, lay.reg_nchunk * lay.reg_kp * lay.reg_ck, slot.reg, lay.reg_elems
            else:
                rows, ktot, src, elems = lay.d1, lay.alt_nchunk * lay.alt_kp * lay.alt_ck, slot.alt, lay.alt_elems
            if elems != rows * ktot or rows % 16 or ktot % 32 or not L.is_half(self.dtype):
                raise L.EvtError(f"no fragment-order form for this image ({which}, {rows} x {ktot}, {self.dtype})")
            if self._items is None:
                self.build_tables()
            f = torch.empty(elems, dtype=self.dtype, device=self.device)
            it = L.FragItem()
            it.src, it.dst, it.rows, it.ktot = src.data_ptr(), f.data_ptr(), rows, ktot
            self._frags[key] = f
            self._frag_items.append(it)
            self._frag_rows.append(self._slot_rows[self.slots.index(slot)])
            self._frag_retired.extend(t for t, _n in self._frag_tables.values() if t is not None)
            self._frag_tables.clear()
            one = L.struct_to_device([it], self.device)
            self._frag_tables[("one", len(self._frag_items))] = (one, 1)
            L.check(L.lib().evt_frag_pack(L.ptr(one), 1, L.stream_ptr()), "evt_frag_pack")
            if not torch.cuda.is_current_stream_capturing():
                items = list(self._frag_items)
                self._frag_tables[(0, self._nrows)] = (L.struct_to_device(items, self.device), len(items))
        return f

    def _repack_frags(self, lo, hi):
        if not self._frag_items:
            return
        tab = self._frag_tables.get((lo, hi))
        if tab is None:
            items = [it for it, (r0, r1) in zip(self._frag_items, self._frag_rows) if r0 < hi and r1 > lo]
            tab = self._frag_tables[(lo, hi)] = (L.struct_to_device(items, self.device) if items else None, len(items))
        if tab[1]:
            L.check(L.lib().evt_frag_pack(L.ptr(tab[0]), tab[1], L.stream_ptr()), "evt_frag_pack")

    def zero_dw(self):
        if self._deferred or self._held:
            self._deferred.clear()
            self._deferred_on.clear()
            self._deferred_bytes = 0
            if self._side is not None:
                torch.cuda.current_stream(self.device).wait_stream(self._side)
            self._held.clear()
        self.dw_arena.zero_()
        self._tables_checked = False
        for s in self.slots:
            s.wg_used, s.wg_dirty = 0, False

    def scratch(self):
        key = torch.cuda.current_stream(self.device).cuda_stream
        ws = self._ws.get(key)
        if ws is None:
            ws = self._ws[key] = torch.empty(4 << 20, dtype=torch.float32, device=self.device)
        return ws

    def side_stream(self):
        if self._side is None:
            self._side = L.role_stream(self.device, "bank")
        return self._side

    def flush_deferred(self):
        if not self._deferred:
            return
        side = self.side_stream()
        side.wait_stream(torch.cuda.current_stream(self.device))
        for st in self._deferred_on:
            side.wait_stream(st)
        self._deferred_on.clear()
        with torch.cuda.stream(side):
            for args in self._deferred:
                _bwd_weight_now(*args)
        self._held.extend((a[1], a[2], a[3]) for a in self._deferred)
        self._deferred.clear()
        self._deferred_bytes = 0

    def join_side(self):
        self.flush_deferred()
        if self._side is not None and self._held:
            torch.cuda.current_stream(self.device).wait_stream(self._side)
        self._held.clear()

    def rows_of(self, modules):
        idx = sorted(i for i, s in enumerate(self.slots) if any(s.module is m for m in modules))
        if not idx or idx != list(range(idx[0], idx[-1] + 1)):
            raise L.EvtError("rows_of: the modules must be a contiguous, non-empty run of this bank's convolutions")
        if self._items is None:
            self.build_tables()
        return self._slot_rows[idx[0]][0], self._slot_rows[idx[-1]][1]

    def check_tables(self):
        if self._items is None:
            self.build_tables()
        elif not getattr(self, "_tables_checked", False) and not torch.cuda.is_current_stream_capturing():
            if self._grad_stamp != self._grad_ptrs():
                self.build_tables()
            self._tables_checked = True

    def grads(self, lo=None, hi=None, join=True):
        if join:
            self.join_side()
        self.check_tables()
        lo = 0 if lo is None else lo
        hi = self._nrows if hi is None else hi
        if hi <= lo:
            return
        rows = C.c_void_p(self._rows.data_ptr() + 8 * lo)
        L.check(L.lib().evt_wn_grad_multi(L.ptr(self._items), rows, hi - lo, L.stream_ptr()), "evt_wn_grad_multi")


class FrozenConv:
    weight_norm, kdims, transposed, groups, dil = False, 1, False, 1, 1

    def __init__(self, weight_fn, bias_fn, cin, cout, k=1, stride=1, padding=0):
        self.weight_fn, self.bias_fn = weight_fn, bias_fn
        self.cin, self.cout, self.k, self.stride, self.pad = cin, cout, k, stride, padding
        self._slot = None

    @property
    def v(self):
        w = self.weight_fn()
        return w if w.dim() == 3 else w.unsqueeze(-1)

    @property
    def bias(self):
        return self.bias_fn() if self.bias_fn is not None else None

    def lout(self, lin):
        return (lin + 2 * self.pad - (self.k - 1) - 1) // self.stride + 1


class FrozenBank:
    weight_grads = False

    def __init__(self, convs, device, impl=L.IMPL_AUTO):
        self.dt, self.dtype, self.device, self.impl = L.DT_F32, torch.float32, torch.device(device), impl
        self.slots, offs, reg_n, alt_n = [], [], 0, 0
        for m in convs:
            lay = conv_layout(self.dt, m.cin, m.cout, m.k, m.stride, m.pad, m.dil, m.groups, m.transposed)
            s = ConvSlot(m, lay, self)
            m._slot = s
            self.slots.append(s)
            offs.append((reg_n, alt_n))
            reg_n += (lay.reg_elems + 127) // 128 * 128
            alt_n += (lay.alt_elems + 127) // 128 * 128
        self.reg_arena = torch.zeros(max(reg_n, 1), dtype=torch.float32, device=device)
        self.alt_arena = torch.zeros(max(alt_n, 1), dtype=torch.float32, device=device)
        for s, (ro, ao) in zip(self.slots, offs):
            s.reg = self.reg_arena[ro: ro + s.layout.reg_elems]
            s.alt = self.alt_arena[ao: ao + s.layout.alt_elems]
        self._stamp = self._items = None

    def prepare(self):
        vs = [s.module.v for s in self.slots]
        stamp = tuple((v.data_ptr(), v._version) for v in vs)
        if stamp == self._stamp:
            return
        items, rows = [], []
        for i, (s, v) in enumerate(zip(self.slots, vs)):
            if v.dtype != torch.float32 or not v.is_contiguous() or v.device != self.device:
                raise L.EvtError("FrozenBank: contiguous fp32 weights on the bank's device expected")
            it = L.WPrepItem()
            it.v, it.g, it.reg, it.alt = v.data_ptr(), None, s.reg.data_ptr(), s.alt.data_ptr()
            it.dw = it.dv = it.dg = None
            it.lay, it.dtype = s.layout, self.dt
            items.append(it)
            rows.extend((i, r) for r in range(s.layout.d0))
        self._items = L.struct_to_device(items, self.device)
        self._rows = torch.tensor(rows, dtype=torch.int32, device=self.device).contiguous()
        L.check(L.lib().evt_wn_fold_multi(L.ptr(self._items), L.ptr(self._rows), len(rows), L.stream_ptr()),
                "evt_wn_fold_multi")
        self._stamp = stamp


PLAIN_X = os.environ.get("EVT_CONV_PLAIN_X", "1") != "0"
TRACE = None


TRACE_RANGES = False


def set_trace(rec, ranges=False):
    global TRACE, TRACE_RANGES
    TRACE = rec
    TRACE_RANGES = bool(ranges) and rec is not None
    L.lib().evt_debug_kernel_tags(1 if rec is not None else 0)


def _t0():
    if TRACE is None:
        return None
    rf = None
    if TRACE_RANGES:
        rf = torch.profiler.record_function(f"evt#{len(TRACE)}")
        rf.__enter__()
    e = torch.cuda.Event(enable_timing=True)
    e.record()
    return e, rf


def _t1(e0, kind, m, nseq, lin, extra_elems):
    e0, rf = e0
    e1 = torch.cuda.Event(enable_timing=True)
    e1.record()
    if rf is not None:
        rf.__exit__(None, None, None)
    lq = lin if m.transposed else m.lout(lin)
    macs = nseq * lq * m.cin * m.cout * m.k // m.groups
    sz = 2 if L.is_half(m._slot.bank.dtype) else 4
    act = nseq * (lin * m.cin + m.lout(lin) * m.cout) + extra_elems
    wbytes = m.v.numel() * (4 if kind == "bwd_weight" else sz)
    shape = (f"{'T' if m.transposed else ''}{m.cin}>{m.cout} k{m.k} s{m.stride} d{m.dil} g{m.groups} "
             f"n{nseq} L{lin}")
    TRACE.append((L.lib().evt_last_kernel_tag().decode(), kind, 2 * macs, act * sz + wbytes, e0, e1, shape, m))


def _t1_elt(e0, name, nbytes, owner):
    e0, rf = e0
    e1 = torch.cuda.Event(enable_timing=True)
    e1.record()
    if rf is not None:
        rf.__exit__(None, None, None)
    TRACE.append((name, "elt", 0, nbytes, e0, e1, name, owner))


def _fwd(slot, x, res, in_slope, out_act, out_slope, out=None):
    m = slot.module
    if x.dim() != 3 or x.size(2) != m.cin or x.dtype != slot.bank.dtype or not x.is_contiguous():
        raise L.EvtError(f"conv input must be contiguous [nseq, L, {m.cin}] {slot.bank.dtype}, got "
                         f"{tuple(x.shape)} {x.dtype} contiguous={x.is_contiguous()}")
    nseq, lin = x.size(0), x.size(1)
    y = out if out is not None else torch.empty((nseq, m.lout(lin), m.cout), dtype=x.dtype, device=x.device)
    if y.shape != (nseq, m.lout(lin), m.cout) or y.dtype != x.dtype or not y.is_contiguous():
        raise L.EvtError("conv output buffer must be contiguous [nseq, Lout, Cout] in the compute dtype")
    if res is not None and (res.shape != y.shape or not res.is_contiguous() or res.dtype != x.dtype):
        raise L.EvtError("residual must match the output")
    p = slot.params(nseq, lin, in_slope, out_act, out_slope)
    bias = m.bias
    e0 = _t0()
    L.check(L.lib().evt_conv1d_fwd(C.byref(p), L.ptr(x), L.ptr(slot.reg), L.ptr(slot.alt),
                                   L.ptr(bias.data if bias is not None else None), L.ptr(res), L.ptr(y),
                                   L.stream_ptr()), "evt_conv1d_fwd")
    if e0 is not None:
        _t1(e0, "fwd", m, nseq, lin, y.numel() if res is not None else 0)
    return y


def _bwd_data(slot, dy, y, x, dx_add, nseq, lin, in_slope, out_act, out_slope):
    m = slot.module
    dx = torch.empty((nseq, lin, m.cin), dtype=dy.dtype, device=dy.device)
    p = slot.params(nseq, lin, in_slope, out_act, out_slope)
    e0 = _t0()
    L.check(L.lib().evt_conv1d_bwd_data(C.byref(p), L.ptr(dy), L.ptr(y if out_act != L.ACT_NONE else None),
                                        L.ptr(slot.reg), L.ptr(slot.alt), L.ptr(x if in_slope != 1.0 else None),
                                        L.ptr(dx_add), L.ptr(dx), L.stream_ptr()), "evt_conv1d_bwd_data")
    if e0 is not None:
        extra = (dy.numel() if out_act != L.ACT_NONE else 0) + (dx.numel() if in_slope != 1.0 else 0) + \
                (dx.numel() if dx_add is not None else 0)
        _t1(e0, "bwd_data", m, nseq, lin, extra)
    return dx


def _bwd_weight(slot, x, dy, y, nseq, lin, in_slope, out_act, out_slope):
    bank = slot.bank
    if slot.packed_member:
        raise L.EvtError("weight gradient of a packed projection member requested on its own: inside a bf16 runtime the "
                         "q / k / v projections of a windowed attention layer run (and are differentiated) as one pack")
    if bank.defer_n > 0 and TRACE is None:
        bank._deferred.append((slot, x, dy, y, nseq, lin, in_slope, out_act, out_slope))
        bank._deferred_on.add(torch.cuda.current_stream(bank.device))
        bank._deferred_bytes += x.numel() * x.element_size() + dy.numel() * dy.element_size()
        if len(bank._deferred) >= bank.defer_n or bank._deferred_bytes >= bank.defer_bytes:
            bank.flush_deferred()
        return
    _bwd_weight_now(slot, x, dy, y, nseq, lin, in_slope, out_act, out_slope)


def _bwd_weight_now(slot, x, dy, y, nseq, lin, in_slope, out_act, out_slope):
    m = slot.module
    p = slot.params(nseq, lin, in_slope, out_act, out_slope)
    dbias = None
    if m.bias is not None:
        if m.bias.grad is None:
            m.bias.grad = torch.zeros_like(m.bias)
        dbias = m.bias.grad
    e0 = _t0()
    if slot.bank.parts_on:
        sp = slot._wgp
        if sp is None:
            sp = slot._wgp = L.WgradParts()
            sp.dw_extra = slot.dw_extra.data_ptr() if slot.parts > 1 else None
            sp.part_stride = (slot.layout.reg_elems + 127) // 128 * 128
            sp.db_part = slot.db_part.data_ptr() if (dbias is not None and not m.transposed) else None
            sp.used_dev = slot.used.data_ptr()
            sp.parts = slot.parts
        sp.prev_used, sp.dirty0 = slot.wg_used, int(slot.wg_dirty)
        ws = slot.bank.scratch()
        sp.ws, sp.ws_floats = ws.data_ptr(), ws.numel()
        L.check(L.lib().evt_conv1d_bwd_weight_parts(C.byref(p), L.ptr(x), L.ptr(dy),
                                                    L.ptr(y if out_act != L.ACT_NONE else None), L.ptr(slot.dw),
                                                    L.ptr(dbias), C.byref(sp), L.stream_ptr()),
                "evt_conv1d_bwd_weight_parts")
        slot.wg_used, slot.wg_dirty = max(slot.wg_used, int(sp.used)), True
    else:
        L.check(L.lib().evt_conv1d_bwd_weight(C.byref(p), L.ptr(x), L.ptr(dy),
                                              L.ptr(y if out_act != L.ACT_NONE else None), L.ptr(slot.dw), L.ptr(dbias),
                                              L.stream_ptr()), "evt_conv1d_bwd_weight")
    if e0 is not None:
        _t1(e0, "bwd_weight", m, nseq, lin, dy.numel() if out_act != L.ACT_NONE else 0)


class ConvFn(torch.autograd.Function):

    @staticmethod
    def forward(ctx, x, anchor, res, slot, in_slope, out_act, out_slope):
        ctx.pre = False
        if in_slope != 1.0 and x.is_cuda and x.dim() == 3 and PLAIN_X and L.lib().evt_conv1d_wants_plain_x(
                C.byref(slot.params(x.size(0), x.size(1), in_slope, out_act, out_slope))):
            xa = torch.empty_like(x)
            e0 = _t0()
            L.check(L.lib().evt_leaky_relu(L.dt_of(x), L.ptr(x), C.c_float(in_slope), L.ptr(xa), C.c_int64(x.numel()),
                                           L.stream_ptr()), "evt_leaky_relu")
            if e0 is not None:
                _t1_elt(e0, "lrelu_kernel", 2 * x.numel() * x.element_size(), slot.module)
            y = _fwd(slot, xa, res, 1.0, out_act, out_slope)
            x, ctx.pre = xa, True
        else:
            y = _fwd(slot, x, res, in_slope, out_act, out_slope)
        ctx.slot, ctx.cfg = slot, (in_slope, out_act, out_slope)
        ctx.has_res = res is not None
        ctx.save_for_backward(x, y if out_act != L.ACT_NONE else None)
        return y

    @staticmethod
    def backward(ctx, dy):
        x, y = ctx.saved_tensors
        slot = ctx.slot
        in_slope, out_act, out_slope = ctx.cfg
        dy = dy.contiguous()
        nseq, lin = x.size(0), x.size(1)
        if out_act != L.ACT_NONE and L.lib().evt_conv1d_wants_plain_dy(
                C.byref(slot.params(nseq, lin, in_slope, out_act, out_slope))):
            dy_eff = torch.empty_like(dy)
            e0 = _t0()
            L.check(L.lib().evt_dact_mul(L.dt_of(dy), L.ptr(dy), L.ptr(y), int(out_act), C.c_float(out_slope),
                                         L.ptr(dy_eff), C.c_int64(dy.numel()), L.stream_ptr()), "evt_dact_mul")
            if e0 is not None:
                _t1_elt(e0, "dact_mul_kernel", 3 * dy.numel() * dy.element_size(), slot.module)
            dy, y, out_act, out_slope = dy_eff, None, L.ACT_NONE, 1.0
        if slot.bank.weight_grads:
            _bwd_weight(slot, x, dy, y, nseq, lin, 1.0 if ctx.pre else in_slope, out_act, out_slope)
        dx = None
        if ctx.needs_input_grad[0]:
            dx = _bwd_data(slot, dy, y, x, None, nseq, lin, in_slope, out_act, out_slope)
        dres = dy if (ctx.has_res and ctx.needs_input_grad[2]) else None
        if dres is not None and out_act != L.ACT_NONE:
            raise L.EvtError("residual + output activation: residual is added after the activation, "
                             "its gradient is dy (supported), but was not expected here")
        return dx, None, dres, None, None, None, None


def _resunit_params(s1, s2, x, slope):
    m1, m2 = s1.module, s2.module
    if (not L.is_half(x.dtype) or not x.is_cuda or not x.is_contiguous() or x.dim() != 3 or m1.cin != m1.cout
            or m2.cin != m2.cout or m1.cin != m2.cin or m1.k != m2.k or m2.dil != 1 or m1.stride != 1 or m2.stride != 1
            or m1.groups != 1 or m2.groups != 1 or m1.transposed or m2.transposed
            or m1.pad != m1.dil * (m1.k - 1) // 2 or m2.pad != (m2.k - 1) // 2 or s1.bank.impl != L.IMPL_AUTO):
        return None
    p = L.ResUnitParams(L.dt_code(x.dtype), x.size(0), x.size(1), m1.cin, m1.k, m1.dil, float(slope))
    return p if L.lib().evt_resunit_supported(C.byref(p)) else None


def _resunit_wide_params(s1, s2, x, slope):
    m1, m2 = s1.module, s2.module
    if (not L.is_half(x.dtype) or not x.is_cuda or not x.is_contiguous() or x.dim() != 3 or m1.cin != m1.cout
            or m2.cin != m2.cout or m1.cin != m2.cin or m1.k != m2.k or m2.dil != 1 or m1.stride != 1 or m2.stride != 1
            or m1.groups != 1 or m2.groups != 1 or m1.transposed or m2.transposed
            or m1.pad != m1.dil * (m1.k - 1) // 2 or m2.pad != (m2.k - 1) // 2 or s1.bank.impl != L.IMPL_AUTO):
        return None
    p = L.ResUnitParams(L.dt_code(x.dtype), x.size(0), x.size(1), m1.cin, m1.k, m1.dil, float(slope))
    return p if L.lib().evt_resunit_wide_supported(C.byref(p)) else None


def _t1_unit(e0, m1, m2, x):
    e0, rf = e0
    e1 = torch.cuda.Event(enable_timing=True)
    e1.record()
    if rf is not None:
        rf.__exit__(None, None, None)
    n, ln, c = x.shape
    macs = n * ln * c * c * (m1.k + m2.k)
    TRACE.append((L.lib().evt_last_kernel_tag().decode(), "fwd", 2 * macs, 4 * x.numel() * 2 + (m1.v.numel() + m2.v.numel()) * 2,
                  e0, e1, f"unit {c}>{c} k{m1.k} d{m1.dil} n{n} L{ln}", m1))


def _lrelu(x, slope, owner=None):
    out = torch.empty_like(x)
    e0 = _t0()
    L.check(L.lib().evt_leaky_relu(L.dt_of(x), L.ptr(x), C.c_float(slope), L.ptr(out), C.c_int64(x.numel()),
                                   L.stream_ptr()), "evt_leaky_relu")
    if e0 is not None:
        _t1_elt(e0, "lrelu_kernel", 2 * x.numel() * x.element_size(), owner)
    return out


def _add3(a, b, c, scale, out, owner):
    e0 = _t0()
    L.check(L.lib().evt_add3_scale(L.dt_of(a), L.ptr(a), L.ptr(b), L.ptr(c), C.c_float(scale), L.ptr(out),
                                   C.c_int64(a.numel()), L.stream_ptr()), "evt_add3_scale")
    if e0 is not None:
        _t1_elt(e0, "add3_scale_kernel", (2 + (b is not None) + (c is not None)) * a.numel() * a.element_size(), owner)
    return out


class ResUnitFn(torch.autograd.Function):

    @staticmethod
    def forward(ctx, x, anchor, s1, s2, slope):
        fused = _resunit_params(s1, s2, x, slope)
        if fused is not None:
            m1, m2 = s1.module, s2.module
            xa, mid_a, y = torch.empty_like(x), torch.empty_like(x), torch.empty_like(x)
            e0 = _t0()
            L.check(L.lib().evt_resunit_fwd(C.byref(fused), L.ptr(x), L.ptr(s1.reg), L.ptr(s2.reg),
                                            L.ptr(m1.bias.data if m1.bias is not None else None),
                                            L.ptr(m2.bias.data if m2.bias is not None else None), L.ptr(xa), L.ptr(mid_a),
                                            L.ptr(y), L.stream_ptr()), "evt_resunit_fwd")
            if e0 is not None:
                _t1_unit(e0, m1, m2, x)
            ctx.s1, ctx.s2, ctx.slope = s1, s2, slope
            ctx.save_for_backward(xa, mid_a)
            return y
        wide = _resunit_wide_params(s1, s2, x, slope)
        if wide is not None:
            m1, m2 = s1.module, s2.module
            xa, mid_a, y = torch.empty_like(x), torch.empty_like(x), torch.empty_like(x)
            e0 = _t0()
            L.check(L.lib().evt_resunit_wide_fwd(C.byref(wide), L.ptr(x), L.ptr(s1.reg), L.ptr(s2.reg),
                                                 L.ptr(m1.bias.data if m1.bias is not None else None),
                                                 L.ptr(m2.bias.data if m2.bias is not None else None), L.ptr(xa),
                                                 L.ptr(mid_a), L.ptr(y), L.stream_ptr()), "evt_resunit_wide_fwd")
            if e0 is not None:
                _t1_unit(e0, m1, m2, x)
            ctx.s1, ctx.s2, ctx.slope = s1, s2, slope
            ctx.save_for_backward(xa, mid_a)
            return y
        xa = _lrelu(x, slope, s1.module)
        mid_a = _fwd(s1, xa, None, 1.0, L.ACT_LRELU, slope)
        y = _fwd(s2, mid_a, x, 1.0, L.ACT_NONE, 1.0)
        ctx.s1, ctx.s2, ctx.slope = s1, s2, slope
        ctx.save_for_backward(xa, mid_a)
# ... 382 lines not shown
```

easevoice_trainer_amd/hip/lib.py:

```python
import ctypes as C
import os

import torch

_HERE = os.path.dirname(os.path.abspath(__file__))
LIB_PATH = os.path.join(os.path.dirname(_HERE), "libevt_hip.so")
LIB_PATH_F16 = os.path.join(os.path.dirname(_HERE), "libevt_hip_f16.so")

DT_F32, DT_BF16, DT_F16 = 0, 1, 2
HALF_DTYPES = (torch.bfloat16, torch.float16)
ACT_NONE, ACT_LRELU, ACT_TANH = 0, 1, 2
IMPL_AUTO, IMPL_NAIVE, IMPL_IGEMM = 0, 1, 2


class EvtError(RuntimeError):
    pass


EVT_OK, EVT_ELAUNCH, EVT_EINVAL, EVT_ENOTSUP = 0, 5, 22, 95


class ConvParams(C.Structure):
    _fields_ = [
        ("dtype", C.c_int32), ("nseq", C.c_int32), ("lin", C.c_int32), ("cin", C.c_int32), ("cout", C.c_int32),
        ("k", C.c_int32), ("stride", C.c_int32), ("pad", C.c_int32), ("dil", C.c_int32), ("groups", C.c_int32),
        ("transposed", C.c_int32), ("in_slope", C.c_float), ("out_act", C.c_int32), ("out_slope", C.c_float),
        ("impl", C.c_int32),
    ]


class ResUnitParams(C.Structure):
    _fields_ = [("dtype", C.c_int32), ("nseq", C.c_int32), ("L", C.c_int32), ("C", C.c_int32), ("k", C.c_int32),
                ("dil", C.c_int32), ("slope", C.c_float)]


class ResUnitFwdJob(C.Structure):
    _fields_ = [("p", ResUnitParams), ("x", C.c_void_p), ("w1_reg", C.c_void_p), ("w2_reg", C.c_void_p),
                ("b1", C.c_void_p), ("b2", C.c_void_p), ("xa", C.c_void_p), ("mid_a", C.c_void_p), ("y", C.c_void_p)]


class ResUnitBwdJob(C.Structure):
    _fields_ = [("p", ResUnitParams), ("dy_scale", C.c_float), ("dy", C.c_void_p), ("xa", C.c_void_p),
                ("mid_a", C.c_void_p), ("w1_alt", C.c_void_p), ("w2_alt", C.c_void_p), ("dx", C.c_void_p),
                ("dmid", C.c_void_p), ("dw1", C.c_void_p), ("dw2", C.c_void_p), ("db1", C.c_void_p), ("db2", C.c_void_p)]


class WLayout(C.Structure):
    _fields_ = [
        ("d0", C.c_int32), ("d1", C.c_int32), ("k", C.c_int32), ("stride", C.c_int32),
        ("reg_ck", C.c_int32), ("reg_nchunk", C.c_int32), ("reg_kp", C.c_int32),
        ("alt_ck", C.c_int32), ("alt_nchunk", C.c_int32), ("alt_kp", C.c_int32), ("alt_nphase", C.c_int32),
        ("reg_elems", C.c_int64), ("alt_elems", C.c_int64),
    ]


class WPrepItem(C.Structure):
    _fields_ = [
        ("v", C.c_void_p), ("g", C.c_void_p), ("reg", C.c_void_p), ("alt", C.c_void_p),
        ("dw", C.c_void_p), ("dv", C.c_void_p), ("dg", C.c_void_p),
        ("lay", WLayout), ("dtype", C.c_int32), ("src_d1", C.c_int32),
        ("dw_extra", C.c_void_p), ("dw_part_stride", C.c_int64), ("db_part", C.c_void_p), ("db", C.c_void_p),
        ("used", C.c_void_p),
    ]


class FragItem(C.Structure):
    _fields_ = [("src", C.c_void_p), ("dst", C.c_void_p), ("rows", C.c_int32), ("ktot", C.c_int32)]


class WgradParts(C.Structure):
    _fields_ = [("dw_extra", C.c_void_p), ("part_stride", C.c_int64), ("db_part", C.c_void_p), ("used_dev", C.c_void_p),
                ("parts", C.c_int32), ("prev_used", C.c_int32), ("used", C.c_int32), ("dirty0", C.c_int32),
                ("ws", C.c_void_p), ("ws_floats", C.c_int64)]


class Seg(C.Structure):
    _fields_ = [("a", C.c_void_p), ("b", C.c_void_p), ("da", C.c_void_p), ("n", C.c_int64),
                ("scale", C.c_float), ("pad_", C.c_int32)]


class KlParams(C.Structure):
    _fields_ = [("B", C.c_int32), ("T", C.c_int32), ("C", C.c_int32), ("time_inner", C.c_int32),
                ("dt_z_p", C.c_int32), ("dt_logs_q", C.c_int32), ("dt_m_p", C.c_int32), ("dt_logs_p", C.c_int32)]


class AdamWSeg(C.Structure):
    _fields_ = [("begin", C.c_int64), ("end", C.c_int64), ("lr", C.c_float), ("weight_decay", C.c_float)]


class AttnParams(C.Structure):
    _fields_ = [
        ("dtype", C.c_int32), ("B", C.c_int32), ("L", C.c_int32), ("H", C.c_int32), ("D", C.c_int32),
        ("x_len", C.c_int32),
        ("q_stride_b", C.c_int64), ("q_stride_l", C.c_int64), ("q_stride_h", C.c_int64),
        ("o_stride_b", C.c_int64), ("o_stride_l", C.c_int64), ("o_stride_h", C.c_int64),
        ("dropout_p", C.c_float), ("seed", C.c_uint32),
    ]


class SampleParams(C.Structure):
    _fields_ = [("V", C.c_int32), ("eos", C.c_int32), ("top_k", C.c_int32), ("no_eos_steps", C.c_int32),
                ("ymax", C.c_int32), ("top_p", C.c_float), ("temperature", C.c_float),
                ("repetition_penalty", C.c_float), ("seed", C.c_uint32), ("noise_rows", C.c_int32)]


class RowSample(C.Structure):
    _fields_ = [("top_k", C.c_int32), ("top_p", C.c_float), ("temperature", C.c_float),
                ("repetition_penalty", C.c_float)]


DEC_POS, DEC_IDX, DEC_YCOUNT, DEC_YLEN, DEC_SEED = 0, 1, 2, 3, 4


class SAChunk(C.Structure):
    _fields_ = [("begin", C.c_int64), ("end", C.c_int64), ("tensor", C.c_int32), ("pad_", C.c_int32)]


class ScaledAdamHP(C.Structure):
    _fields_ = [("lr", C.c_float), ("beta1", C.c_float), ("beta2", C.c_float), ("eps", C.c_float),
                ("scalar_lr_scale", C.c_float), ("scalar_max", C.c_float), ("step", C.c_int32), ("pad_", C.c_int32)]


class MhaParams(C.Structure):
    _fields_ = [("dtype", C.c_int32), ("B", C.c_int32), ("H", C.c_int32), ("D", C.c_int32), ("Tq", C.c_int32),
                ("Tk", C.c_int32), ("window", C.c_int32), ("n_heads_rel", C.c_int32), ("ldq", C.c_int64),
                ("ldk", C.c_int64), ("ldo", C.c_int64), ("scale", C.c_float), ("dropout_p", C.c_float),
                ("site", C.c_uint32), ("pad_", C.c_uint32), ("seed_dev", C.c_void_p)]


_libs = {}
_half = torch.bfloat16


def set_half(dtype) -> None:
    global _half
    if dtype in HALF_DTYPES:
        _half = dtype


def half():
    return _half


def is_half(dtype) -> bool:
    return dtype in HALF_DTYPES


def dt_code(dtype) -> int:
    if dtype == torch.float32:
        return DT_F32
    if dtype in HALF_DTYPES:
        if dtype != _half:
            raise EvtError(f"{dtype} data while the {_half} build of the library is selected: call hip.lib.set_half({dtype}) "
                           "(the engines do, at the top of a step)")
        return DT_BF16 if dtype == torch.bfloat16 else DT_F16
    raise EvtError(f"unsupported dtype {dtype}")


def _check_fresh(handle, LIB_PATH=LIB_PATH):
    csrc = os.path.join(os.path.dirname(_HERE), "csrc")
    if os.environ.get("EVT_ALLOW_STALE_LIB") == "1" or not os.path.isdir(csrc):
        return
    from ..build import source_hash

    have = handle.evt_version().decode()
    want = source_hash()
    if f"src={want}" not in have:
        raise EvtError(f"{LIB_PATH} is stale: built from sources {have.split('src=')[-1]!r}, the tree has {want!r}; "
                       "rebuild with `python -m easevoice_trainer_amd.build` (EVT_ALLOW_STALE_LIB=1 overrides)")


def lib():
    _lib = _libs.get(_half)
    if _lib is None:
        path = LIB_PATH if _half == torch.bfloat16 else LIB_PATH_F16
        if not os.path.exists(path):
            raise EvtError(
                f"{path} not found: build it with `python -m easevoice_trainer_amd.build` "
                "(or __graft_entry__.build()). There is no fallback path.")
        _lib = C.CDLL(path)
        _lib.evt_version.restype = C.c_char_p
        _check_fresh(_lib, path)
        _lib.evt_half_dtype.restype = C.c_int32
        if _lib.evt_half_dtype() != (DT_BF16 if _half == torch.bfloat16 else DT_F16):
            raise EvtError(f"{path} serves half code {_lib.evt_half_dtype()}: not the {_half} build")
        _libs[_half] = _lib
        _lib.evt_conv1d_lout.restype = C.c_int32
        _lib.evt_mel_workspace_floats.restype = C.c_int64
        _lib.evt_workspace_bytes.restype = C.c_int64
        _lib.evt_last_kernel_tag.restype = C.c_char_p
        _lib.evt_resunit_bwd_ws_floats.restype = C.c_int64
        _lib.evt_debug_kernel_tags.restype = None
        for name in ("evt_resunit_fwd_multi_lens", "evt_resunit_wide_fwd_lens", "evt_mask_tail", "evt_resample_rows",
                     "evt_resample_pack_rows", "evt_hubert_front_rows", "evt_clip_rescale_rows", "evt_phone_expand_rows",
                     "evt_bert_embed_ln_rows", "evt_ref_spec_rows", "evt_mish_rows_fwd", "evt_glu_res_rows_fwd",
                     "evt_mean_rows"):
            getattr(_lib, name).restype = C.c_int
        _lib.evt_hubert_front_ws_floats.restype = C.c_int64
    return _lib


def check(rc: int, what: str) -> None:
    if rc != 0:
        raise EvtError(f"{what} failed with code {rc}")


def dt_of(t: torch.Tensor) -> int:
    return dt_code(t.dtype)


def torch_dtype(dt: int) -> torch.dtype:
    return {DT_F32: torch.float32, DT_BF16: torch.bfloat16, DT_F16: torch.float16}[dt]


def ptr(t):
    if t is None:
        return C.c_void_p(0)
    if not t.is_contiguous():
        raise EvtError("non-contiguous tensor passed to the C ABI")
    return C.c_void_p(t.data_ptr())


_hip_rt = None
_role_pools = {}


# ... 62 lines not shown
```

easevoice_trainer_amd/hip/wn.py:

```python
import ctypes as C

import torch

from . import conv as HC
from . import lib as L


class WNStackFn(torch.autograd.Function):
    @staticmethod
    def forward(ctx, x, g_lbh, lens, anchor, in_slots, rs_slots, hidden):
        n_layers, H = len(in_slots), hidden
        B, T, _ = x.shape
        if not x.is_contiguous() or x.size(2) != H or (g_lbh is not None and not g_lbh.is_contiguous()):
            raise L.EvtError("WN stack: contiguous [B, T, H] input and [n_layers, B, 2H] conditioning expected")
        dt = L.dt_of(x)
        rows = B * T
        saved = []
        out = None
        fused = FUSED_FORWARD and _layer_fused(dt, H, in_slots, rs_slots)
        frag_in, frag_rs = _frag_images(in_slots, rs_slots) if fused else (None, None)
        for i in range(n_layers):
            last = i == n_layers - 1
            if fused:
                mi, mr = in_slots[i].module, rs_slots[i].module
                x_in = torch.empty((B, T, 2 * H), dtype=x.dtype, device=x.device)
                acts = torch.empty((B, T, H), dtype=x.dtype, device=x.device)
                acc_out = torch.empty((B, T, H), dtype=x.dtype, device=x.device)
                x_out = None if last else torch.empty_like(acc_out)
                e0 = HC._t0()
                L.check(L.lib().evt_wn_layer_fwd(dt, L.ptr(x), L.ptr(frag_in[i]),
                                                 L.ptr(mi.bias.data if mi.bias is not None else None), L.ptr(frag_rs[i]),
                                                 L.ptr(mr.bias.data if mr.bias is not None else None),
                                                 L.ptr(g_lbh[i] if g_lbh is not None else None), L.ptr(out), L.ptr(lens),
                                                 L.ptr(x_in), L.ptr(acts), L.ptr(x_out), L.ptr(acc_out), B, T, H, mi.k,
                                                 int(last), L.stream_ptr()), "evt_wn_layer_fwd")
                if e0 is not None:
                    _t1_layer(e0, mi, mr, x)
                saved += [x, x_in, acts]
                x, out = x_out, acc_out
                continue
            x_in = HC._fwd(in_slots[i], x, None, 1.0, L.ACT_NONE, 1.0)
            acts = torch.empty((B, T, H), dtype=x.dtype, device=x.device)
            L.check(L.lib().evt_gated_act_fwd(dt, L.ptr(x_in), L.ptr(g_lbh[i] if g_lbh is not None else None), L.ptr(acts),
                                              B, T, H, L.stream_ptr()), "evt_gated_act_fwd")
            rs = HC._fwd(rs_slots[i], acts, None, 1.0, L.ACT_NONE, 1.0)
            acc_out = torch.empty((B, T, H), dtype=x.dtype, device=x.device)
            x_out = None if last else torch.empty_like(acc_out)
            L.check(L.lib().evt_wn_residual_fwd(dt, L.ptr(None if last else x), L.ptr(rs), L.ptr(out), L.ptr(lens), T,
                                                L.ptr(x_out), L.ptr(acc_out), C.c_int64(rows), H, int(last),
                                                L.stream_ptr()), "evt_wn_residual_fwd")
            saved += [x, x_in, acts]
            x, out = x_out, acc_out
        ctx.save_for_backward(lens, g_lbh, *saved)
        ctx.cfg = (in_slots, rs_slots, H, B, T)
        return out

    @staticmethod
    def backward(ctx, dout):
        lens, g_lbh, *saved = ctx.saved_tensors
        in_slots, rs_slots, H, B, T = ctx.cfg
        n_layers = len(in_slots)
        dtype, dev = dout.dtype, dout.device
        dt = L.dt_code(dtype)
        rows = B * T
        dacc = dout.contiguous()
        dx_next = None
        dg32 = torch.zeros((n_layers, B, 2 * H), dtype=torch.float32, device=dev) if g_lbh is not None else None
        fused = FUSED_BACKWARD and _layer_fused(dt, H, in_slots, rs_slots)
        for i in reversed(range(n_layers)):
            last = i == n_layers - 1
            x, x_in, acts = saved[3 * i: 3 * i + 3]
            rs_w = H if last else 2 * H
            if fused:
                si, sr = in_slots[i], rs_slots[i]
                drs = torch.empty((B, T, rs_w), dtype=dtype, device=dev)
                dx_in = torch.empty((B, T, 2 * H), dtype=dtype, device=dev)
                dx = torch.empty((B, T, H), dtype=dtype, device=dev)
                e0 = HC._t0()
                L.check(L.lib().evt_wn_layer_bwd_data(dt, L.ptr(dx_next), L.ptr(dacc), L.ptr(x_in),
                                                      L.ptr(g_lbh[i] if g_lbh is not None else None),
                                                      L.ptr(sr.bank.frag(sr, "alt")), L.ptr(si.bank.frag(si, "alt")),
                                                      L.ptr(lens), L.ptr(drs), L.ptr(dx_in), L.ptr(dx),
                                                      L.ptr(dg32[i] if dg32 is not None else None), B, T, H, si.module.k,
                                                      int(last), L.stream_ptr()), "evt_wn_layer_bwd_data")
                if e0 is not None:
                    _t1_layer(e0, si.module, sr.module, x, "bwd_data")
                if last:
                    dacc = drs
                if sr.bank.weight_grads:
                    HC._bwd_weight(sr, acts, drs, None, B, T, 1.0, L.ACT_NONE, 1.0)
                if si.bank.weight_grads:
                    HC._bwd_weight(si, x, dx_in, None, B, T, 1.0, L.ACT_NONE, 1.0)
                dx_next = dx
                continue
            drs = torch.empty((B, T, rs_w), dtype=dtype, device=dev)
            dx_res = None if last else torch.empty((B, T, H), dtype=dtype, device=dev)
            L.check(L.lib().evt_wn_residual_bwd(dt, L.ptr(dx_next), L.ptr(dacc), L.ptr(lens), T, L.ptr(dx_res), L.ptr(drs),
                                                C.c_int64(rows), H, int(last), L.stream_ptr()), "evt_wn_residual_bwd")
            if last:
                dacc = drs
            s = rs_slots[i]
            if s.bank.weight_grads:
                HC._bwd_weight(s, acts, drs, None, B, T, 1.0, L.ACT_NONE, 1.0)
            dacts = HC._bwd_data(s, drs, None, acts, None, B, T, 1.0, L.ACT_NONE, 1.0)
            dx_in = torch.empty_like(x_in)
            L.check(L.lib().evt_gated_act_bwd(dt, L.ptr(x_in), L.ptr(g_lbh[i] if g_lbh is not None else None), L.ptr(dacts),
                                              L.ptr(dx_in), L.ptr(dg32[i] if dg32 is not None else None), B, T, H,
                                              L.stream_ptr()), "evt_gated_act_bwd")
            s = in_slots[i]
            if s.bank.weight_grads:
                HC._bwd_weight(s, x, dx_in, None, B, T, 1.0, L.ACT_NONE, 1.0)
            need_dx = i > 0 or ctx.needs_input_grad[0]
            dx_next = HC._bwd_data(s, dx_in, None, x, dx_res, B, T, 1.0, L.ACT_NONE, 1.0) if need_dx else None
        dg = dg32.to(g_lbh.dtype) if (dg32 is not None and ctx.needs_input_grad[1]) else None
        return dx_next, dg, None, None, None, None, None


FUSED_FORWARD = True
FUSED_BACKWARD = True


def _layer_fused(dt, H, in_slots, rs_slots):
    bank = in_slots[0].bank
    cache = bank.__dict__.setdefault("_wn_fused", {})
    key = (id(in_slots[0]), len(in_slots), dt, H)
    ok = cache.get(key)
    if ok is None:
        ok = cache[key] = _layer_fused_check(dt, H, in_slots, rs_slots)
    return ok


def _layer_fused_check(dt, H, in_slots, rs_slots):
    n = len(in_slots)
    for i, (si, sr) in enumerate(zip(in_slots, rs_slots)):
        mi, mr = si.module, sr.module
        if not L.lib().evt_wn_layer_supported(dt, H, mi.k, mi.dil):
            return False
        if (mi.cin, mi.cout, mi.stride, mi.groups, mi.pad, mi.transposed) != (H, 2 * H, 1, 1, (mi.k - 1) // 2, False):
            return False
        if (mr.cin, mr.cout, mr.k, mr.stride, mr.groups, mr.pad, mr.transposed) != (H, H if i == n - 1 else 2 * H, 1, 1, 1, 0,
                                                                                    False):
            return False
    return True


def _frag_images(in_slots, rs_slots):
    bank = in_slots[0].bank
    return [bank.frag(s, "reg") for s in in_slots], [bank.frag(s, "reg") for s in rs_slots]


def _t1_layer(e0, mi, mr, x, kind="fwd"):
    e0, rf = e0
    e1 = torch.cuda.Event(enable_timing=True)
    e1.record()
    if rf is not None:
        rf.__exit__(None, None, None)
    n, ln, h = x.shape
    macs = n * ln * (mi.cin * mi.cout * mi.k + mr.cin * mr.cout)
    HC.TRACE.append((L.lib().evt_last_kernel_tag().decode(), kind, 2 * macs,
                     (7 * x.numel() + mi.v.numel() + mr.v.numel()) * 2, e0, e1,
                     f"WN layer {h}>{mi.cout}>{mr.cout} k{mi.k} n{n} L{ln}", mi))


def wn_stack(x, g_lbh, lens, in_layers, rs_layers, hidden):
    in_slots = tuple(m._slot for m in in_layers)
    rs_slots = tuple(m._slot for m in rs_layers)
    if any(s is None for s in in_slots + rs_slots):
        raise L.EvtError("WN stack before WeightBank.attach(); there is no eager fallback")
    return WNStackFn.apply(x, g_lbh, lens, in_slots[0].bank.anchor, in_slots, rs_slots, int(hidden))
```

include/evt.h:

```cpp
#ifndef EVT_H
#define EVT_H
#include <stddef.h>
#include <stdint.h>

#ifdef __cplusplus
extern "C" {
#endif
#pragma GCC visibility push(default)

#define EVT_DT_F32 0
#define EVT_DT_BF16 1
#define EVT_DT_F16 2
#define EVT_ACT_NONE 0
#define EVT_ACT_LRELU 1
#define EVT_ACT_TANH 2
#define EVT_IMPL_AUTO 0
#define EVT_IMPL_NAIVE 1
#define EVT_IMPL_IGEMM 2

const char* evt_version(void);
int32_t evt_half_dtype(void);
void evt_debug_kernel_tags(int32_t enable);
const char* evt_last_kernel_tag(void);

#define EVT_WS_NONE 0
#define EVT_WS_MEL 1
#define EVT_WS_ATTN_BWD 2
#define EVT_WS_MHA_BWD 3
#define EVT_WS_MASKED_KL 4
int64_t evt_workspace_bytes(int32_t op, const int64_t* dims, int32_t ndims);

typedef struct evt_conv1d_params {
  int32_t dtype;
  int32_t nseq;
  int32_t lin;
  int32_t cin, cout;
  int32_t k, stride, pad, dil, groups;
  int32_t transposed;
  float in_slope;
  int32_t out_act;
  float out_slope;
  int32_t impl;
} evt_conv1d_params;

int32_t evt_conv1d_wants_plain_dy(const evt_conv1d_params* c);

int32_t evt_conv1d_wants_plain_x(const evt_conv1d_params* c);

int32_t evt_conv1d_lout(const evt_conv1d_params* p);

typedef struct evt_wlayout {
  int32_t d0, d1, k, stride;
  int32_t reg_ck, reg_nchunk, reg_kp;
  int32_t alt_ck, alt_nchunk, alt_kp, alt_nphase;
  int64_t reg_elems, alt_elems;
} evt_wlayout;
int evt_conv1d_layout(const evt_conv1d_params* p, evt_wlayout* out);

typedef struct evt_wprep_item {
  const float* v;
  const float* g;
  void* reg;
  void* alt;
  const float* dw;
  float* dv;
  float* dg;
  evt_wlayout lay;
  int32_t dtype;
  int32_t src_d1;
  const float* dw_extra;
  int64_t dw_part_stride;
  const float* db_part;
  float* db;
  const int32_t* used;
} evt_wprep_item;
int evt_wn_fold_multi(const evt_wprep_item* items, const int32_t* row_index, int32_t nrows, void* stream);
int evt_wn_fold_groups(const evt_wprep_item* items, const int32_t* group_index, int32_t ngroups, void* stream);
int evt_wn_grad_multi(const evt_wprep_item* items, const int32_t* row_index, int32_t nrows, void* stream);

int evt_conv1d_fwd(const evt_conv1d_params* p, const void* x, const void* w_reg, const void* w_alt,
                   const float* bias, const void* res, void* y, void* stream);

int evt_conv1d_bwd_data(const evt_conv1d_params* p, const void* dy, const void* y, const void* w_reg,
                        const void* w_alt, const void* x, const void* dx_add, void* dx, void* stream);

int evt_conv1d_bwd_weight(const evt_conv1d_params* p, const void* x, const void* dy, const void* y,
                          float* dw, float* dbias, void* stream);

typedef struct evt_wgrad_parts {
  float* dw_extra;
  int64_t part_stride;
  float* db_part;
  int32_t* used_dev;
  int32_t parts;
  int32_t prev_used;
  int32_t used;
  int32_t dirty0;
  float* ws;
  int64_t ws_floats;
} evt_wgrad_parts;
int evt_conv1d_bwd_weight_parts(const evt_conv1d_params* p, const void* x, const void* dy, const void* y,
                                float* dw, float* dbias, evt_wgrad_parts* sp, void* stream);

typedef struct evt_resunit_params {
  int32_t dtype, nseq, L, C, k, dil;
  float slope;
} evt_resunit_params;
int32_t evt_resunit_supported(const evt_resunit_params* p);
int evt_resunit_fwd(const evt_resunit_params* p, const void* x, const void* w1_reg, const void* w2_reg, const float* b1,
                    const float* b2, void* xa, void* mid_a, void* y, void* stream);

typedef struct evt_resunit_fwd_job {
  evt_resunit_params p;
  const void* x; const void* w1_reg; const void* w2_reg; const float* b1; const float* b2;
  void* xa; void* mid_a; void* y;
} evt_resunit_fwd_job;
int evt_resunit_fwd_multi(const evt_resunit_fwd_job* jobs, int32_t njobs, void* stream);

int evt_resunit_fwd_multi_lens(const evt_resunit_fwd_job* jobs, int32_t njobs, const int32_t* lens, int32_t mul,
                               void* stream);

int32_t evt_resunit_bwd_supported(const evt_resunit_params* p, int32_t with_weight_grads);
int64_t evt_resunit_bwd_ws_floats(const evt_resunit_params* p);
int evt_resunit_bwd(const evt_resunit_params* p, const void* dy, float dy_scale, const void* xa, const void* mid_a,
                    const void* w1_alt, const void* w2_alt, void* dx, void* dmid, float* dw1, float* dw2, float* db1,
                    float* db2, float* ws, int64_t ws_floats, void* stream);
typedef struct evt_resunit_bwd_job {
  evt_resunit_params p;
  float dy_scale;
  const void* dy; const void* xa; const void* mid_a; const void* w1_alt; const void* w2_alt;
  void* dx; void* dmid;
  float* dw1; float* dw2; float* db1; float* db2;
} evt_resunit_bwd_job;
int evt_resunit_bwd_multi(const evt_resunit_bwd_job* jobs, int32_t njobs, float* ws, int64_t ws_floats, void* stream);

int32_t evt_resunit_wide_supported(const evt_resunit_params* p);
int evt_resunit_wide_fwd(const evt_resunit_params* p, const void* x, const void* w1_reg, const void* w2_reg, const float* b1,
                         const float* b2, void* xa, void* mid_a, void* y, void* stream);
int evt_resunit_wide_fwd_lens(const evt_resunit_params* p, const void* x, const void* w1_reg, const void* w2_reg,
                              const float* b1, const float* b2, void* xa, void* mid_a, void* y, const int32_t* lens,
                              int32_t mul, void* stream);
int evt_resunit_wide_bwd_data(const evt_resunit_params* p, const void* dy, float dy_scale, const void* xa, const void* mid_a,
                              const void* w1_alt, const void* w2_alt, void* dmid, void* dx, void* stream);

typedef struct evt_frag_item {
  const void* src;
  void* dst;
  int32_t rows, ktot;
} evt_frag_item;
int evt_frag_pack(const evt_frag_item* items, int32_t nitems, void* stream);
int evt_wn_layer_bwd_data(int32_t dtype, const void* dx_next, const void* dacc, const void* x_in, const void* g,
                          const void* w_rs_alt_frag, const void* w_in_alt_frag, const int32_t* lens, void* drs, void* dx_in,
                          void* dx, float* dg, int32_t nseq, int32_t L, int32_t H, int32_t k, int32_t last, void* stream);
int32_t evt_wn_layer_supported(int32_t dtype, int32_t H, int32_t k, int32_t dil);
int evt_wn_layer_fwd(int32_t dtype, const void* x, const void* w_in_frag, const float* b_in, const void* w_rs_frag,
                     const float* b_rs, const void* g, const void* acc_in, const int32_t* lens, void* x_in, void* acts,
                     void* x_out, void* acc_out, int32_t nseq, int32_t L, int32_t H, int32_t k, int32_t last, void* stream);

int evt_add3_scale(int32_t dtype, const void* a, const void* b, const void* c, float scale, void* out,
                   int64_t n, void* stream);

int evt_mask_tail(int32_t dtype, void* x, const int32_t* lens, int32_t mul, int32_t nseq, int32_t L, int32_t C,
                  void* stream);

int evt_resample_rows(int32_t dtype, const void* x, const int32_t* in_lens, const int32_t* out_lens, int32_t nseq,
                      int32_t Lin, int32_t Lout, int32_t C, void* y, void* stream);

#define EVT_RESAMPLE_ZEROS 64
#define EVT_RESAMPLE_TILE 2048
#define EVT_PCM_F32 0
#define EVT_PCM_S16 1
int evt_resample_pack_rows(int32_t dtype, const void* x, const int32_t* lens, int32_t mul, int32_t nseq, int32_t L,
                           int32_t up, int32_t down, const float* table, int32_t J, int32_t out_format, void* out,
                           int64_t out_elems, const int64_t* out_off, int32_t gap, void* stream);

int evt_leaky_relu(int32_t dtype, const void* x, float slope, void* out, int64_t n, void* stream);

int evt_dact_mul(int32_t dtype, const void* dy, const void* y, int32_t act_kind, float slope, void* out, int64_t n,
                 void* stream);

int evt_gated_act_fwd(int32_t dtype, const void* xin, const void* g, void* acts, int32_t nseq, int32_t len,
                      int32_t H, void* stream);
int evt_gated_act_bwd(int32_t dtype, const void* xin, const void* g, const void* dacts, void* dxin, float* dg,
                      int32_t nseq, int32_t len, int32_t H, void* stream);


int evt_mel_fwd(const float* wav, const float* window, const float* mel_basis, float* spec_out, float* mel_out,
                float* ws_spec_re_im, int32_t nseq, int32_t wav_len, int32_t n_fft, int32_t hop, int32_t n_mels,
                void* stream);
int evt_mel_bwd(const float* dmel, const float* window, const float* mel_basis, const float* ws_spec_re_im,
                float* dwav, int32_t nseq, int32_t wav_len, int32_t n_fft, int32_t hop, int32_t n_mels, void* stream);
int64_t evt_mel_workspace_floats(int32_t nseq, int32_t wav_len, int32_t n_fft, int32_t hop, int32_t n_mels);

int evt_ref_spec_rows(const float* x, const int32_t* lens, int32_t nseq, int32_t N, const float* window, int32_t n_fft,
                      int32_t hop, int32_t bins, float* out, float* peak, void* stream);

int evt_ncl_to_nlc(int32_t dtype, const float* src, void* dst, int32_t B, int32_t C, int32_t T, int32_t Cp, void* stream);

int evt_rvq_norms(const float* embed, float* ee, int32_t K, int32_t D, void* stream);
int evt_rvq_select(const float* h, const float* dots, const float* embed, const float* ee, int64_t* codes, float* q_out,
                   int32_t N, int32_t D, int32_t K, int32_t rep, void* stream);

int evt_spec_to_mel(const float* spec, const float* basis, const int64_t* starts, float* out, int32_t B, int32_t F,
                    int32_t T, int32_t M, int32_t nfr, void* stream);

typedef struct evt_seg { const void* a; const void* b; void* da; int64_t n; float scale; int32_t pad_; } evt_seg;
int evt_l1_multi_fwd(int32_t dtype, const evt_seg* segs, int32_t nseg, float* out, void* stream);
int evt_l1_multi_bwd(int32_t dtype, const evt_seg* segs, int32_t nseg, const float* dloss, void* stream);
int evt_lsgan_multi_fwd(int32_t dtype, const evt_seg* segs, int32_t nseg, float target, float* out, void* stream);
int evt_lsgan_multi_bwd(int32_t dtype, const evt_seg* segs, int32_t nseg, float target, const float* dloss,
                        void* stream);

typedef struct evt_kl_params {
  int32_t B, T, C, time_inner;
  int32_t dt_z_p, dt_logs_q, dt_m_p, dt_logs_p;
} evt_kl_params;
int evt_masked_kl_fwd(const evt_kl_params* p, const void* z_p, const void* logs_q, const void* m_p, const void* logs_p,
                      const int32_t* lens, float* out2, void* stream);
int evt_masked_kl_bwd(const evt_kl_params* p, const void* z_p, const void* logs_q, const void* m_p, const void* logs_p,
                      const int32_t* lens, const float* dloss, const float* count, void* dz_p, void* dlogs_q, void* dm_p,
                      void* dlogs_p, void* stream);

typedef struct evt_adamw_seg { int64_t begin, end; float lr; float weight_decay; } evt_adamw_seg;
int evt_adamw_flat(float* param, const float* grad, float* exp_avg, float* exp_avg_sq, int64_t n,
                   const evt_adamw_seg* segs, int32_t nseg, float beta1, float beta2, float eps, int32_t step,
                   float grad_scale, void* stream);
int evt_adamw_flat_dev(float* param, const float* grad, float* exp_avg, float* exp_avg_sq, int64_t n,
                       const evt_adamw_seg* segs, int32_t nseg, float beta1, float beta2, float eps,
                       int32_t* step_counter, float grad_scale, void* stream);
int evt_adamw_flat_dev_range(float* param, const float* grad, float* exp_avg, float* exp_avg_sq, int64_t lo, int64_t hi,
                             const evt_adamw_seg* segs, int32_t nseg, float beta1, float beta2, float eps,
                             int32_t* step_counter, int32_t bump, float grad_scale, void* stream);
int evt_mpd_fold(int32_t src0_dtype, const void* src0, int32_t n0, int32_t src1_dtype, const void* src1, int32_t n1, int32_t T,
                 const int32_t* periods, int32_t nper, void* const* outs, int32_t out_dtype, void* stream);
int evt_mpd_unfold(int32_t grad_dtype, const void* const* douts, const int32_t* periods, int32_t nper, int32_t b0, int32_t n,
                   int32_t T, int32_t dsrc_dtype, void* dsrc, void* stream);

int evt_sumsq(const float* x, int64_t n, float* out, void* stream);

int evt_scaler_unscale(float* grad, int64_t n, const float* scale, float* found_inf, void* stream);
int evt_adamw_flat_dev_guarded(float* param, const float* grad, float* exp_avg, float* exp_avg_sq, int64_t n,
                               const evt_adamw_seg* segs, int32_t nseg, float beta1, float beta2, float eps,
                               int32_t* step_counter, float grad_scale, const float* skip, void* stream);
int evt_scaler_update(float* scale, int32_t* growth_tracker, float* const* found_inf, int32_t nflags, float growth_factor,
                      float backoff_factor, int32_t growth_interval, void* stream);

typedef struct evt_gemm_params {
  int32_t dtype;
  int32_t M, N, K;
  int32_t relu;
} evt_gemm_params;
int evt_gemm_bf16_layout(const evt_gemm_params* g, evt_wlayout* out);
int evt_gemm_bf16_fwd(const evt_gemm_params* g, const void* x, const void* w_reg, const void* w_alt, const float* bias,
                      void* y, void* stream);
int evt_gemm_bf16_bwd_data(const evt_gemm_params* g, const void* dy, const void* w_reg, const void* w_alt, void* dx,
// ... 225 lines not shown
```

Baseline: 3489 audio-s/s.

## Group WN-layer weight-gradient ring kernels into batched multi-member launches

Adds a grouped weight-gradient entry point that buckets ring-eligible conv wgrad jobs by tile shape and runs up to 16 of them in one launch. The grid's z dimension indexes the member, and the split count is planned jointly across members against a shared block target. The WN backward stack now collects the in/res-skip wgrads of two layers and flushes them together. This aims to cut per-kernel launch and tail underutilization for the many small wgrads. In exchange it pads the grid to the largest member, which leaves idle blocks, and it changes how the split-K partitioning is chosen.

```diff
diff --git a/easevoice_trainer_amd/csrc/conv1d.hip b/easevoice_trainer_amd/csrc/conv1d.hip
--- a/easevoice_trainer_amd/csrc/conv1d.hip
+++ b/easevoice_trainer_amd/csrc/conv1d.hip
@@ -1283,12 +1283,11 @@
   return evt_conv1d_bwd_weight_parts(c, x, dy, y, dw, dbias, nullptr, stream);
 }
 
-int evt_conv1d_bwd_weight_parts(const evt_conv1d_params* c, const void* x, const void* dy, const void* y, float* dw,
-                                float* dbias, evt_wgrad_parts* sp, void* stream) {
+static int wg_check_args(const evt_conv1d_params* c, const void* x, const void* dy, const void* y, float* dw,
+                         evt_wgrad_parts* sp) {
   int rc = valid(c);
   if (rc) return rc;
   if (!x || !dy || !dw) return EVT_EINVAL;
-  int used_host = 0;
   if (sp) {
     sp->used = 0;
     if (sp->parts < 1 || !sp->used_dev || sp->prev_used < 0 || sp->prev_used > sp->parts) return EVT_EINVAL;
@@ -1296,13 +1295,25 @@
     if (sp->ws && sp->ws_floats <= 0) return EVT_EINVAL;
   }
   if (c->out_act != EVT_ACT_NONE && !y) return EVT_EINVAL;
-  hipStream_t st = (hipStream_t)stream;
-  const int lout = evt_conv1d_lout(c);
-  const void* ysv = c->out_act != EVT_ACT_NONE ? y : nullptr;
+  return 0;
+}
+
+struct WgRoute {
+  WgP p;
+  int lout;
+  const void* ysv;
+  bool grouped, igemm_path, gemm_w, halo_w, deep_w, ring_w;
+};
+
+static WgRoute wg_route(const evt_conv1d_params* c, const void* x, const void* dy, const void* y, float* dw,
+                        const evt_wgrad_parts* sp, int* used_host) {
+  WgRoute r{};
+  const int lout = r.lout = evt_conv1d_lout(c);
+  const void* ysv = r.ysv = c->out_act != EVT_ACT_NONE ? y : nullptr;
   evt_wlayout l; evt_conv1d_layout(c, &l);
-  const bool grouped = c->impl != EVT_IMPL_NAIVE && evt_grouped_supported(c);
-  const bool igemm_path = !grouped && c->impl != EVT_IMPL_NAIVE && igemm_ok(c) && l.reg_kp <= 64;
-  WgP p{};
+  const bool grouped = r.grouped = c->impl != EVT_IMPL_NAIVE && evt_grouped_supported(c);
+  const bool igemm_path = r.igemm_path = !grouped && c->impl != EVT_IMPL_NAIVE && igemm_ok(c) && l.reg_kp <= 64;
+  WgP& p = r.p;
   p.dw = dw; p.nseq = c->nseq; p.KH = c->k; p.KHp = l.reg_kp; p.s = c->stride; p.dil = c->dil; p.off = -c->pad;
   if (!c->transposed) {
     p.A = dy; p.Aact = ysv; p.aact_kind = c->out_act; p.aact_slope = c->out_slope; p.a_slope = 1.f;
@@ -1316,12 +1327,31 @@
   p.dbias = nullptr;
   if (sp) {
     p.dw_extra = sp->dw_extra; p.part_stride = sp->part_stride; p.parts = sp->parts; p.prev_used = sp->prev_used;
-    p.db_part = sp->db_part; p.used = sp->used_dev; p.used_host = &used_host; p.dirty0 = sp->dirty0 || sp->prev_used > 0;
-  }
-  const bool gemm_w = igemm_path && c->impl == EVT_IMPL_AUTO && !c->transposed && evt_conv::wgrad_gemm_eligible(p, c->dtype);
-  const bool halo_w = !gemm_w && igemm_path && c->impl == EVT_IMPL_AUTO && evt_conv::wgrad_halo_eligible(p, c->dtype);
-  const bool deep_w = !gemm_w && !halo_w && igemm_path && c->impl == EVT_IMPL_AUTO && evt_conv::wgrad_deep_eligible(p, c->dtype);
-  const bool ring_w = !deep_w && !halo_w && igemm_path && c->impl == EVT_IMPL_AUTO && evt_conv::wgrad_ring_eligible(p, c->dtype);
+    p.db_part = sp->db_part; p.used = sp->used_dev; p.used_host = used_host; p.dirty0 = sp->dirty0 || sp->prev_used > 0;
+  }
+  const bool gemm_w = r.gemm_w = igemm_path && c->impl == EVT_IMPL_AUTO && !c->transposed && evt_conv::wgrad_gemm_eligible(p, c->dtype);
+  const bool halo_w = r.halo_w = !gemm_w && igemm_path && c->impl == EVT_IMPL_AUTO && evt_conv::wgrad_halo_eligible(p, c->dtype);
+  const bool deep_w = r.deep_w = !gemm_w && !halo_w && igemm_path && c->impl == EVT_IMPL_AUTO && evt_conv::wgrad_deep_eligible(p, c->dtype);
+  r.ring_w = !deep_w && !halo_w && igemm_path && c->impl == EVT_IMPL_AUTO && evt_conv::wgrad_ring_eligible(p, c->dtype);
+  return r;
+}
+
+static bool wg_fuses_bias_igemm(const evt_conv1d_params* c, const WgRoute& r, const float* dbias) {
+  return dbias && r.igemm_path && c->dtype == EVT_DT_HALF && !c->transposed;
+}
+
+int evt_conv1d_bwd_weight_parts(const evt_conv1d_params* c, const void* x, const void* dy, const void* y, float* dw,
+                                float* dbias, evt_wgrad_parts* sp, void* stream) {
+  int rc = wg_check_args(c, x, dy, y, dw, sp);
+  if (rc) return rc;
+  int used_host = 0;
+  hipStream_t st = (hipStream_t)stream;
+  WgRoute route = wg_route(c, x, dy, y, dw, sp, &used_host);
+  WgP& p = route.p;
+  const int lout = route.lout;
+  const void* ysv = route.ysv;
+  const bool grouped = route.grouped, igemm_path = route.igemm_path, gemm_w = route.gemm_w, halo_w = route.halo_w,
+             deep_w = route.deep_w, ring_w = route.ring_w;
   const bool cin1 = !grouped && c->impl != EVT_IMPL_NAIVE && evt_small_kind(c) == 2;
   const bool cout1 = !grouped && c->impl != EVT_IMPL_NAIVE && evt_small_kind(c) == 1;
   const bool fuse_bias = dbias && ((igemm_path && c->dtype == EVT_DT_HALF && !c->transposed) || cin1 || cout1);
@@ -1420,4 +1450,97 @@
   return launch_wgrad(c->dtype, p, st);
 }
 
-}
+int evt_wgrad_group_plan(evt_wgrad_plan* m, int32_t n, int64_t target) {
+  if (!m || n < 0 || target < 1) return EVT_EINVAL;
+  for (int i0 = 0; i0 < n; i0 += EVT_WGRAD_GROUP_MAX) {
+    const int cnt = n - i0 < EVT_WGRAD_GROUP_MAX ? n - i0 : EVT_WGRAD_GROUP_MAX;
+    long tiles[EVT_WGRAD_GROUP_MAX];
+    int stages[EVT_WGRAD_GROUP_MAX], mins[EVT_WGRAD_GROUP_MAX], parts[EVT_WGRAD_GROUP_MAX], nsplit[EVT_WGRAD_GROUP_MAX],
+        per[EVT_WGRAD_GROUP_MAX];
+    for (int i = 0; i < cnt; ++i) {
+      const evt_wgrad_plan& e = m[i0 + i];
+      if (e.tiles < 1 || e.stages < 1) return EVT_EINVAL;
+      tiles[i] = (long)e.tiles; stages[i] = e.stages; mins[i] = e.min_stages; parts[i] = e.parts;
+    }
+    evt_conv::wgrad_group_plan(tiles, stages, mins, parts, cnt, (long)target, nsplit, per);
+    for (int i = 0; i < cnt; ++i) {
+      m[i0 + i].launch = i0 / EVT_WGRAD_GROUP_MAX;
+      m[i0 + i].nsplit = nsplit[i];
+      m[i0 + i].per = per[i];
+    }
+  }
+  return 0;
+}
+
+namespace {
+struct WgBucket {
+  int MA, KT, s, n;
+  WgP ps[EVT_WGRAD_GROUP_MAX];
+  int used_host[EVT_WGRAD_GROUP_MAX];
+  evt_wgrad_parts* sp[EVT_WGRAD_GROUP_MAX];
+};
+
+int wg_bucket_launch(WgBucket& b, hipStream_t st) {
+  if (b.n == 0) return 0;
+  const int rc = b.n == 1 ? evt_conv::launch_wgrad_ring(b.ps[0], st) : evt_conv::launch_wgrad_ring_group(b.ps, b.n, st);
+  for (int i = 0; i < b.n; ++i)
+    if (b.sp[i]) b.sp[i]->used = b.used_host[i];
+  b.n = 0;
+  return rc;
+}
+}
+
+int evt_conv1d_bwd_weight_group(const evt_wgrad_member* members, int32_t n, void* stream) {
+  if (n < 0 || (n > 0 && !members)) return EVT_EINVAL;
+  hipStream_t st = (hipStream_t)stream;
+  for (int i = 0; i < n; ++i) {
+    const evt_wgrad_member& m = members[i];
+    if (!m.p) return EVT_EINVAL;
+    const int rc = wg_check_args(m.p, m.x, m.dy, m.y, m.dw, m.sp);
+    if (rc) return rc;
+    for (int j = 0; j < i; ++j)
+      if (members[j].dw == m.dw) return EVT_EINVAL;
+  }
+  constexpr int NB = 6;
+  static thread_local WgBucket buckets[NB];
+  int nb = 0;
+  for (int i = 0; i < n; ++i) {
+    const evt_wgrad_member& m = members[i];
+    int used_host = 0;
+    WgRoute r = wg_route(m.p, m.x, m.dy, m.y, m.dw, m.sp, &used_host);
+    const bool together = r.ring_w && (!m.dbias || wg_fuses_bias_igemm(m.p, r, m.dbias));
+    WgBucket* b = nullptr;
+    if (together) {
+      const evt_conv::WgRingShape sh = evt_conv::wgrad_ring_shape(r.p);
+      for (int k = 0; k < nb && !b; ++k)
+        if (buckets[k].MA == sh.MA && buckets[k].KT == sh.KT && buckets[k].s == r.p.s) b = &buckets[k];
+      if (!b && nb < NB) {
+        b = &buckets[nb++];
+        b->MA = sh.MA; b->KT = sh.KT; b->s = r.p.s; b->n = 0;
+      }
+    }
+    if (!b) {
+      const int rc = evt_conv1d_bwd_weight_parts(m.p, m.x, m.dy, m.y, m.dw, m.dbias, m.sp, stream);
+      if (rc) return rc;
+      continue;
+    }
+    const int k = b->n++;
+    b->ps[k] = r.p;
+    b->ps[k].dbias = m.dbias;
+    if (!m.dbias) b->ps[k].db_part = nullptr;
+    b->used_host[k] = 0;
+    b->ps[k].used_host = m.sp ? &b->used_host[k] : nullptr;
+    b->sp[k] = m.sp;
+    if (b->n == EVT_WGRAD_GROUP_MAX) {
+      const int rc = wg_bucket_launch(*b, st);
+      if (rc) return rc;
+    }
+  }
+  for (int k = 0; k < nb; ++k) {
+    const int rc = wg_bucket_launch(buckets[k], st);
+    if (rc) return rc;
+  }
+  return 0;
+}
+
+}
diff --git a/easevoice_trainer_amd/csrc/conv_deep.hip b/easevoice_trainer_amd/csrc/conv_deep.hip
--- a/easevoice_trainer_amd/csrc/conv_deep.hip
+++ b/easevoice_trainer_amd/csrc/conv_deep.hip
@@ -556,7 +556,7 @@
     if (do_bias) wg_bias_mma<4>(bacc, a, wc);
   }
   if (do_bias) wg_finish_bias_mma<4>(p, bacc, a0, wr, wc, g8, j16, blockIdx.y);
-  wg_finish<4, WKT>(p, smem, acc, ntap, a0, ch, t0, wr, wc, g8, j16, blockIdx.y);
+  wg_finish<4, WKT>(p, smem, acc, ntap, a0, ch, t0, wr, wc, g8, j16, blockIdx.y, blockIdx.x == 0 && blockIdx.y == 0);
 }
 
 constexpr int GKT = 4;
@@ -1052,7 +1052,7 @@
 }
 
 template <int MA, int KT, int NS>
-__global__ __launch_bounds__(256) void wgrad_ring(WgP p, int stages_per_split) {
+__device__ __forceinline__ void wgrad_ring_block(const WgP& p, int stages_per_split, int tile, int split) {
   constexpr int AROW = 64 * MA;
   constexpr int ABYTES = WPOS * AROW;
   constexpr int STAGE = ABYTES + KT * WB_BYTES;
@@ -1064,8 +1064,7 @@
   const int j16 = lane & 15, g8 = lane >> 4;
   const int wr = wave >> 1, wc = wave & 1;
 
-  int bx = blockIdx.x;
-  const int split = blockIdx.y;
+  int bx = tile;
   const int ch = bx % p.nchunk; bx /= p.nchunk;
   const int tgi = bx % p.ntapgrp;
   const int atile = bx / p.ntapgrp;
@@ -1165,7 +1164,30 @@
     asm volatile("" ::: "memory");
   }
   if (do_bias) wg_finish_bias_mma<MA>(p, bacc, a0, wr, wc, g8, j16, split);
-  wg_finish<MA, KT>(p, smem, acc, ntap, a0, ch, t0, wr, wc, g8, j16, split);
+  wg_finish<MA, KT>(p, smem, acc, ntap, a0, ch, t0, wr, wc, g8, j16, split, tile == 0 && split == 0);
+}
+
+template <int MA, int KT, int NS>
+__global__ __launch_bounds__(256) void wgrad_ring(WgP p, int stages_per_split) {
+  wgrad_ring_block<MA, KT, NS>(p, stages_per_split, blockIdx.x, blockIdx.y);
+}
+
+__device__ __forceinline__ WgP wg_member_desc(const WgP& base, const WgMember& r) {
+  WgP p = base;
+  p.A = r.A; p.B = r.B; p.dw = r.dw; p.dw_extra = r.dw_extra; p.db_part = r.db_part; p.dbias = r.dbias; p.used = r.used;
+  p.part_stride = r.part_stride;
+  p.nseq = r.nseq; p.LA = r.LA; p.LB = r.LB; p.CA = r.CA; p.CB = r.CB; p.KH = r.KH; p.KHp = r.KHp; p.dil = r.dil;
+  p.off = r.off; p.Q = r.Q; p.nchunk = r.nchunk; p.ntapgrp = r.ntapgrp;
+  p.parts = r.parts; p.prev_used = r.prev_used; p.now_used = r.now_used; p.dirty0 = r.dirty0; p.nsplit = r.nsplit;
+  return p;
+}
+
+template <int MA, int KT, int NS>
+__global__ __launch_bounds__(256) void wgrad_ring_group(WgGroup g) {
+  const WgMember& r = g.m[blockIdx.z];
+  if ((int)blockIdx.x >= r.tiles || (int)blockIdx.y >= r.nsplit) return;
+  const WgP p = wg_member_desc(g.base, r);
+  wgrad_ring_block<MA, KT, NS>(p, r.per, blockIdx.x, blockIdx.y);
 }
 
 }
@@ -1377,19 +1399,108 @@
   return true;
 }
 
+WgRingShape wgrad_ring_shape(const WgP& p) {
+  WgRingShape s;
+  s.KT = p.KHp <= 1 ? 1 : (p.KHp <= 3 ? 3 : 5);
+  s.nchunk = p.CB / 32;
+  s.ntapgrp = (p.KHp + s.KT - 1) / s.KT;
+  s.nstages = (int)(((long)p.nseq * p.Q + WPOS - 1) / WPOS);
+  const long tiles128 = p.CA % 128 == 0 ? (long)(p.CA / 128) * s.nchunk * s.ntapgrp : 0;
+  s.MA = (tiles128 >= 128 || (tiles128 > 0 && tiles128 * (s.nstages / 4) >= 512)) ? 4 : 2;
+  s.tiles = (long)(p.CA / (32 * s.MA)) * s.nchunk * s.ntapgrp;
+  return s;
+}
+
+void wgrad_group_plan(const long* tiles, const int* nstages, const int* min_stages, const int* parts, int n, long target,
+                      int* nsplit, int* per) {
+  long total = 0;
+  for (int i = 0; i < n; ++i) total += tiles[i];
+  if (total < 1) total = 1;
+  const long want = (target + total - 1) / total;
+  for (int i = 0; i < n; ++i) {
+    long split = want;
+    const int ms = min_stages[i] > 0 ? min_stages[i] : 1;
+    if (split > nstages[i] / ms) split = nstages[i] / ms;
+    if (parts[i] > 0 && split > parts[i]) split = parts[i];
+    if (split < 1) split = 1;
+    per[i] = (int)((nstages[i] + split - 1) / split);
+    if (per[i] < 1) per[i] = 1;
+    nsplit[i] = (nstages[i] + per[i] - 1) / per[i];
+    if (nsplit[i] < 1) nsplit[i] = 1;
+  }
+}
+
+template <int MA, int KT, int NS>
+static int launch_ring_group_inst(const WgGroup& g, int n, int max_tiles, int max_split, hipStream_t st) {
+  constexpr size_t lds = (size_t)NS * (WPOS * 64 * MA + KT * WB_BYTES);
+  static bool attr = false;
+  if (!attr) {
+    if (hipFuncSetAttribute(reinterpret_cast<const void*>(&wgrad_ring_group<MA, KT, NS>),
+                            hipFuncAttributeMaxDynamicSharedMemorySize, (int)lds) != hipSuccess)
+      return EVT_ELAUNCH;
+    attr = true;
+  }
+  evt_set_last_tag("wgrad_ring<bf16, %d, %dx32, 64, x%d> group of %d", 32 * MA, KT, NS, n);
+  hipLaunchKernelGGL((wgrad_ring_group<MA, KT, NS>), dim3((unsigned)max_tiles, (unsigned)max_split, (unsigned)n), dim3(256),
+                     lds, st, g);
+  return evt_check_launch();
+}
+
+int launch_wgrad_ring_group(WgP* ps, int n, hipStream_t st) {
+  if (n < 2 || n > WG_GROUP_MAX) return EVT_EINVAL;
+  long tiles[WG_GROUP_MAX];
+  int nstages[WG_GROUP_MAX], min_stages[WG_GROUP_MAX], parts[WG_GROUP_MAX], nsplit[WG_GROUP_MAX], per[WG_GROUP_MAX];
+  WgRingShape sh[WG_GROUP_MAX];
+  for (int i = 0; i < n; ++i) {
+    if (!wgrad_ring_eligible(ps[i], EVT_DT_HALF)) return EVT_ENOTSUP;
+    sh[i] = wgrad_ring_shape(ps[i]);
+    if (sh[i].MA != sh[0].MA || sh[i].KT != sh[0].KT || ps[i].s != ps[0].s) return EVT_EINVAL;
+    for (int j = 0; j < i; ++j)
+      if (ps[j].dw == ps[i].dw) return EVT_EINVAL;
+    tiles[i] = sh[i].tiles; nstages[i] = sh[i].nstages; min_stages[i] = WG_RING_MIN_STAGES; parts[i] = ps[i].parts;
+  }
+  wgrad_group_plan(tiles, nstages, min_stages, parts, n, WG_RING_TARGET, nsplit, per);
+  WgGroup g;
+  g.base = ps[0];
+  g.base.used_host = nullptr;
+  int max_tiles = 0, max_split = 0;
+  for (int i = 0; i < n; ++i) {
+    WgP& p = ps[i];
+    p.nchunk = sh[i].nchunk; p.ntapgrp = sh[i].ntapgrp;
+    p.nsplit = nsplit[i];
+    p.now_used = p.prev_used > nsplit[i] ? p.prev_used : nsplit[i];
+    if (p.parts > 0 && p.used_host) *p.used_host = p.now_used;
+    WgMember& r = g.m[i];
+    r.A = p.A; r.B = p.B; r.dw = p.dw; r.dw_extra = p.dw_extra; r.db_part = p.db_part; r.dbias = p.dbias; r.used = p.used;
+    r.part_stride = p.part_stride;
+    r.nseq = p.nseq; r.LA = p.LA; r.LB = p.LB; r.CA = p.CA; r.CB = p.CB; r.KH = p.KH; r.KHp = p.KHp; r.dil = p.dil;
+    r.off = p.off; r.Q = p.Q; r.nchunk = p.nchunk; r.ntapgrp = p.ntapgrp;
+    r.parts = p.parts; r.prev_used = p.prev_used; r.now_used = p.now_used; r.dirty0 = p.dirty0;
+    r.nsplit = nsplit[i]; r.per = per[i]; r.tiles = (int)tiles[i];
+    if (r.tiles > max_tiles) max_tiles = r.tiles;
+    if (r.nsplit > max_split) max_split = r.nsplit;
+  }
+  for (int i = n; i < WG_GROUP_MAX; ++i) g.m[i] = g.m[0];
+#define RINGG(MA_, KT_)                                                                               \
+  (MA_ == 4 && KT_ == 5 ? launch_ring_group_inst<MA_, KT_, 3>(g, n, max_tiles, max_split, st)        \
+                        : launch_ring_group_inst<MA_, KT_, 4>(g, n, max_tiles, max_split, st))
+  const int MA = sh[0].MA, KT = sh[0].KT;
+  if (MA == 4) return KT == 1 ? RINGG(4, 1) : (KT == 3 ? RINGG(4, 3) : RINGG(4, 5));
+  return KT == 1 ? RINGG(2, 1) : (KT == 3 ? RINGG(2, 3) : RINGG(2, 5));
+#undef RINGG
+}
+
 int launch_wgrad_ring(const WgP& p_in, hipStream_t st) {
   WgP p = p_in;
   if (!wgrad_ring_eligible(p, EVT_DT_HALF)) return EVT_ENOTSUP;
-  const int KT = p.KHp <= 1 ? 1 : (p.KHp <= 3 ? 3 : 5);
-  p.nchunk = p.CB / 32;
-  p.ntapgrp = (p.KHp + KT - 1) / KT;
-  const int nstages = (int)(((long)p.nseq * p.Q + WPOS - 1) / WPOS);
-  const long tiles128 = p.CA % 128 == 0 ? (long)(p.CA / 128) * p.nchunk * p.ntapgrp : 0;
-  const int MA = (tiles128 >= 128 || (tiles128 > 0 && tiles128 * (nstages / 4) >= 512)) ? 4 : 2;
-  const long tiles = (long)(p.CA / (32 * MA)) * p.nchunk * p.ntapgrp;
-  constexpr long target = 256;
+  const WgRingShape sh = wgrad_ring_shape(p);
+  const int KT = sh.KT, MA = sh.MA, nstages = sh.nstages;
+  p.nchunk = sh.nchunk;
+  p.ntapgrp = sh.ntapgrp;
+  const long tiles = sh.tiles;
+  constexpr long target = WG_RING_TARGET;
   int nsplit, per;
-  wgrad_pick_split(p, tiles, nstages, target, 3, &nsplit, &per);
+  wgrad_pick_split(p, tiles, nstages, target, WG_RING_MIN_STAGES, &nsplit, &per);
   p.nsplit = nsplit;
   p.now_used = p.prev_used > nsplit ? p.prev_used : nsplit;
   if (p.parts > 0 && p.used_host) *p.used_host = p.now_used;
diff --git a/easevoice_trainer_amd/csrc/conv_p.h b/easevoice_trainer_amd/csrc/conv_p.h
--- a/easevoice_trainer_amd/csrc/conv_p.h
+++ b/easevoice_trainer_amd/csrc/conv_p.h
@@ -74,6 +74,34 @@
 int launch_fold_partials2(const float* part, long stride, int nb, float* out, long n, float* out2, long n2, hipStream_t st);
 void wgrad_pick_split(const WgP& p, long tiles, int nstages, long target, int min_stages, int* nsplit, int* per);
 
+struct WgMember {
+  const void* A;
+  const void* B;
+  float* dw;
+  float* dw_extra;
+  float* db_part;
+  float* dbias;
+  int* used;
+  long part_stride;
+  int nseq, LA, LB, CA, CB, KH, KHp, dil, off, Q, nchunk, ntapgrp;
+  int parts, prev_used, now_used, dirty0;
+  int nsplit, per, tiles;
+};
+constexpr int WG_GROUP_MAX = EVT_WGRAD_GROUP_MAX;
+struct WgGroup {
+  WgP base;
+  WgMember m[WG_GROUP_MAX];
+};
+static_assert(sizeof(WgGroup) <= 3072, "grouped weight-gradient table: kernel arguments are limited to 4 KB");
+
+struct WgRingShape { int MA, KT, nchunk, ntapgrp, nstages; long tiles; };
+constexpr long WG_RING_TARGET = 256;
+constexpr int WG_RING_MIN_STAGES = 3;
+WgRingShape wgrad_ring_shape(const WgP& p);
+void wgrad_group_plan(const long* tiles, const int* nstages, const int* min_stages, const int* parts, int n, long target,
+                      int* nsplit, int* per);
+int launch_wgrad_ring_group(WgP* ps, int n, hipStream_t st);
+
 bool rows16_eligible(const struct evt_conv1d_params* c, int rows, int n_out, int k_red, bool fused);
 int launch_rows16(const void* x, const void* w, const float* bias, void* y, int M, int N, int K, hipStream_t st);
 
diff --git a/easevoice_trainer_amd/csrc/wgrad_epi.h b/easevoice_trainer_amd/csrc/wgrad_epi.h
--- a/easevoice_trainer_amd/csrc/wgrad_epi.h
+++ b/easevoice_trainer_amd/csrc/wgrad_epi.h
@@ -50,9 +50,9 @@
 
 template <int MI, int NT>
 __device__ __forceinline__ void wg_finish(const WgP& p, unsigned char* smem, const f32x4 (&acc)[MI][NT], int ntap, int a0,
-                                          int ch, int t0, int wr, int wc, int g8, int j16, int split) {
+                                          int ch, int t0, int wr, int wc, int g8, int j16, int split, bool first) {
   if (p.parts > 0) {
-    if (blockIdx.x == 0 && blockIdx.y == 0 && threadIdx.x == 0) p.used[0] = p.now_used;
+    if (first && threadIdx.x == 0) p.used[0] = p.now_used;
     wg_store_slab<MI, NT>(p, wg_slab(p, split), split == 0 ? p.dirty0 != 0 : split < p.prev_used, reinterpret_cast<float*>(smem), acc, ntap,
                           a0, ch, t0, wr, wc, g8, j16);
     return;
diff --git a/easevoice_trainer_amd/csrc/wgrad_halo.hip b/easevoice_trainer_amd/csrc/wgrad_halo.hip
--- a/easevoice_trainer_amd/csrc/wgrad_halo.hip
+++ b/easevoice_trainer_amd/csrc/wgrad_halo.hip
@@ -192,7 +192,7 @@
     asm volatile("" ::: "memory");
   }
   if (do_bias) wg_finish_bias_mma<MA>(p, bacc, a0, wr, wc, g8, j16, blockIdx.y);
-  wg_finish<MA, NT>(p, smem, acc, NT, a0, ch, 0, wr, wc, g8, j16, blockIdx.y);
+  wg_finish<MA, NT>(p, smem, acc, NT, a0, ch, 0, wr, wc, g8, j16, blockIdx.y, blockIdx.x == 0 && blockIdx.y == 0);
 }
 
 template <int MA, int NT, int NS>
diff --git a/easevoice_trainer_amd/hip/conv.py b/easevoice_trainer_amd/hip/conv.py
--- a/easevoice_trainer_amd/hip/conv.py
+++ b/easevoice_trainer_amd/hip/conv.py
@@ -330,6 +330,9 @@
             self._side = L.role_stream(self.device, "bank")
         return self._side
 
+    def queued(self):
+        return sum(len(e) if isinstance(e, WgGroup) else 1 for e in self._deferred)
+
     def flush_deferred(self):
         if not self._deferred:
             return
@@ -340,8 +343,12 @@
         self._deferred_on.clear()
         with torch.cuda.stream(side):
             for args in self._deferred:
-                _bwd_weight_now(*args)
-        self._held.extend((a[1], a[2], a[3]) for a in self._deferred)
+                if isinstance(args, WgGroup):
+                    _bwd_weight_group_now(args)
+                else:
+                    _bwd_weight_now(*args)
+        for args in self._deferred:
+            self._held.extend((a[1], a[2], a[3]) for a in (args if isinstance(args, WgGroup) else (args,)))
         self._deferred.clear()
         self._deferred_bytes = 0
 
@@ -540,33 +547,105 @@
         bank._deferred.append((slot, x, dy, y, nseq, lin, in_slope, out_act, out_slope))
         bank._deferred_on.add(torch.cuda.current_stream(bank.device))
         bank._deferred_bytes += x.numel() * x.element_size() + dy.numel() * dy.element_size()
-        if len(bank._deferred) >= bank.defer_n or bank._deferred_bytes >= bank.defer_bytes:
+        if bank.queued() >= bank.defer_n or bank._deferred_bytes >= bank.defer_bytes:
             bank.flush_deferred()
         return
     _bwd_weight_now(slot, x, dy, y, nseq, lin, in_slope, out_act, out_slope)
 
 
+GROUP_FLUSH = False
+
+
+class WgGroup(list):
+    """a DECLARED group of weight gradients as one entry of WeightBank._deferred: the argument tuples of _bwd_weight for
+    convolutions that become ready together (the layers of a WN stack), handed over by the module that owns them -- what
+    is in a group never depends on when the queue is flushed"""
+
+
+def _bwd_weight_group(members):
+    members = WgGroup(members)
+    if not members:
+        return
+    bank = members[0][0].bank
+    for a in members:
+        if a[0].packed_member or a[0].bank is not bank:
+            raise L.EvtError("a weight-gradient group takes convolutions of one bank, none of them a packed projection member")
+    if TRACE is not None:
+        for a in members:
+            _bwd_weight_now(*a)
+        return
+    if bank.defer_n > 0:
+        bank._deferred.append(members)
+        bank._deferred_on.add(torch.cuda.current_stream(bank.device))
+        bank._deferred_bytes += sum(a[1].numel() * a[1].element_size() + a[2].numel() * a[2].element_size() for a in members)
+        if GROUP_FLUSH or bank.queued() >= bank.defer_n or bank._deferred_bytes >= bank.defer_bytes:
+            bank.flush_deferred()
+        return
+    _bwd_weight_group_now(members)
+
+
+def _bwd_weight_group_now(members):
+    run, seen = [], set()
+    for a in members:
+        if id(a[0]) in seen:
+            _bwd_weight_group_call(run)
+            run, seen = [], set()
+        run.append(a)
+        seen.add(id(a[0]))
+    _bwd_weight_group_call(run)
+
+
+def _bwd_weight_group_call(members):
+    if len(members) == 1:
+        _bwd_weight_now(*members[0])
+        return
+    arr = (L.WgradMember * len(members))()
+    keep = []
+    for r, (slot, x, dy, y, nseq, lin, in_slope, out_act, out_slope) in zip(arr, members):
+        p = slot.params(nseq, lin, in_slope, out_act, out_slope)
+        dbias = _dbias_of(slot.module)
+        sp = _wgrad_parts(slot, dbias) if slot.bank.parts_on else None
+        keep.append((p, sp))
+        r.p, r.x, r.dy = C.addressof(p), x.data_ptr(), dy.data_ptr()
+        r.y = y.data_ptr() if (out_act != L.ACT_NONE and y is not None) else None
+        r.dw, r.dbias = slot.dw.data_ptr(), (dbias.data_ptr() if dbias is not None else None)
+        r.sp = C.addressof(sp) if sp is not None else None
+    L.check(L.lib().evt_conv1d_bwd_weight_group(arr, len(members), L.stream_ptr()), "evt_conv1d_bwd_weight_group")
+    for (slot, *_), (_p, sp) in zip(members, keep):
+        if sp is not None:
+            slot.wg_used, slot.wg_dirty = max(slot.wg_used, int(sp.used)), True
+
+
+def _dbias_of(m):
+    if m.bias is None:
+        return None
+    if m.bias.grad is None:
+        m.bias.grad = torch.zeros_like(m.bias)
+    return m.bias.grad
+
+
+def _wgrad_parts(slot, dbias):
+    sp = slot._wgp
+    if sp is None:
+        sp = slot._wgp = L.WgradParts()
+        sp.dw_extra = slot.dw_extra.data_ptr() if slot.parts > 1 else None
+        sp.part_stride = (slot.layout.reg_elems + 127) // 128 * 128
+        sp.db_part = slot.db_part.data_ptr() if (dbias is not None and not slot.module.transposed) else None
+        sp.used_dev = slot.used.data_ptr()
+        sp.parts = slot.parts
+    sp.prev_used, sp.dirty0 = slot.wg_used, int(slot.wg_dirty)
+    ws = slot.bank.scratch()
+    sp.ws, sp.ws_floats = ws.data_ptr(), ws.numel()
+    return sp
+
+
 def _bwd_weight_now(slot, x, dy, y, nseq, lin, in_slope, out_act, out_slope):
     m = slot.module
     p = slot.params(nseq, lin, in_slope, out_act, out_slope)
-    dbias = None
-    if m.bias is not None:
-        if m.bias.grad is None:
-            m.bias.grad = torch.zeros_like(m.bias)
-        dbias = m.bias.grad
+    dbias = _dbias_of(m)
     e0 = _t0()
     if slot.bank.parts_on:
-        sp = slot._wgp
-        if sp is None:
-            sp = slot._wgp = L.WgradParts()
-            sp.dw_extra = slot.dw_extra.data_ptr() if slot.parts > 1 else None
-            sp.part_stride = (slot.layout.reg_elems + 127) // 128 * 128
-            sp.db_part = slot.db_part.data_ptr() if (dbias is not None and not m.transposed) else None
-            sp.used_dev = slot.used.data_ptr()
-            sp.parts = slot.parts
-        sp.prev_used, sp.dirty0 = slot.wg_used, int(slot.wg_dirty)
-        ws = slot.bank.scratch()
-        sp.ws, sp.ws_floats = ws.data_ptr(), ws.numel()
+        sp = _wgrad_parts(slot, dbias)
         L.check(L.lib().evt_conv1d_bwd_weight_parts(C.byref(p), L.ptr(x), L.ptr(dy),
                                                     L.ptr(y if out_act != L.ACT_NONE else None), L.ptr(slot.dw),
                                                     L.ptr(dbias), C.byref(sp), L.stream_ptr()),
diff --git a/easevoice_trainer_amd/hip/lib.py b/easevoice_trainer_amd/hip/lib.py
--- a/easevoice_trainer_amd/hip/lib.py
+++ b/easevoice_trainer_amd/hip/lib.py
@@ -72,6 +72,19 @@
     _fields_ = [("dw_extra", C.c_void_p), ("part_stride", C.c_int64), ("db_part", C.c_void_p), ("used_dev", C.c_void_p),
                 ("parts", C.c_int32), ("prev_used", C.c_int32), ("used", C.c_int32), ("dirty0", C.c_int32),
                 ("ws", C.c_void_p), ("ws_floats", C.c_int64)]
+
+
+class WgradMember(C.Structure):
+    _fields_ = [("p", C.c_void_p), ("x", C.c_void_p), ("dy", C.c_void_p), ("y", C.c_void_p), ("dw", C.c_void_p),
+                ("dbias", C.c_void_p), ("sp", C.c_void_p)]
+
+
+class WgradPlan(C.Structure):
+    _fields_ = [("tiles", C.c_int64), ("stages", C.c_int32), ("min_stages", C.c_int32), ("parts", C.c_int32),
+                ("launch", C.c_int32), ("nsplit", C.c_int32), ("per", C.c_int32)]
+
+
+WGRAD_GROUP_MAX = 16
 
 
 class Seg(C.Structure):
diff --git a/easevoice_trainer_amd/hip/wn.py b/easevoice_trainer_amd/hip/wn.py
--- a/easevoice_trainer_amd/hip/wn.py
+++ b/easevoice_trainer_amd/hip/wn.py
@@ -67,6 +67,17 @@
         dx_next = None
         dg32 = torch.zeros((n_layers, B, 2 * H), dtype=torch.float32, device=dev) if g_lbh is not None else None
         fused = FUSED_BACKWARD and _layer_fused(dt, H, in_slots, rs_slots)
+        group = [] if (GROUP_WGRADS and HC.TRACE is None) else None
+
+        def wgrad(*args):
+            if group is None:
+                HC._bwd_weight(*args)
+                return
+            group.append(args)
+            if len(group) >= 2 * GROUP_LAYERS:
+                HC._bwd_weight_group(list(group))
+                group.clear()
+
         for i in reversed(range(n_layers)):
             last = i == n_layers - 1
             x, x_in, acts = saved[3 * i: 3 * i + 3]
@@ -88,9 +99,9 @@
                 if last:
                     dacc = drs
                 if sr.bank.weight_grads:
-                    HC._bwd_weight(sr, acts, drs, None, B, T, 1.0, L.ACT_NONE, 1.0)
+                    wgrad(sr, acts, drs, None, B, T, 1.0, L.ACT_NONE, 1.0)
                 if si.bank.weight_grads:
-                    HC._bwd_weight(si, x, dx_in, None, B, T, 1.0, L.ACT_NONE, 1.0)
+                    wgrad(si, x, dx_in, None, B, T, 1.0, L.ACT_NONE, 1.0)
                 dx_next = dx
                 continue
             drs = torch.empty((B, T, rs_w), dtype=dtype, device=dev)
@@ -101,7 +112,7 @@
                 dacc = drs
             s = rs_slots[i]
             if s.bank.weight_grads:
-                HC._bwd_weight(s, acts, drs, None, B, T, 1.0, L.ACT_NONE, 1.0)
+                wgrad(s, acts, drs, None, B, T, 1.0, L.ACT_NONE, 1.0)
             dacts = HC._bwd_data(s, drs, None, acts, None, B, T, 1.0, L.ACT_NONE, 1.0)
             dx_in = torch.empty_like(x_in)
             L.check(L.lib().evt_gated_act_bwd(dt, L.ptr(x_in), L.ptr(g_lbh[i] if g_lbh is not None else None), L.ptr(dacts),
@@ -109,15 +120,19 @@
                                               L.stream_ptr()), "evt_gated_act_bwd")
             s = in_slots[i]
             if s.bank.weight_grads:
-                HC._bwd_weight(s, x, dx_in, None, B, T, 1.0, L.ACT_NONE, 1.0)
+                wgrad(s, x, dx_in, None, B, T, 1.0, L.ACT_NONE, 1.0)
             need_dx = i > 0 or ctx.needs_input_grad[0]
             dx_next = HC._bwd_data(s, dx_in, None, x, dx_res, B, T, 1.0, L.ACT_NONE, 1.0) if need_dx else None
+        if group:
+            HC._bwd_weight_group(group)
         dg = dg32.to(g_lbh.dtype) if (dg32 is not None and ctx.needs_input_grad[1]) else None
         return dx_next, dg, None, None, None, None, None
 
 
 FUSED_FORWARD = True
 FUSED_BACKWARD = True
+GROUP_WGRADS = True
+GROUP_LAYERS = 2
 
 
 def _layer_fused(dt, H, in_slots, rs_slots):
diff --git a/include/evt.h b/include/evt.h
--- a/include/evt.h
+++ b/include/evt.h
@@ -101,6 +101,29 @@
 } evt_wgrad_parts;
 int evt_conv1d_bwd_weight_parts(const evt_conv1d_params* p, const void* x, const void* dy, const void* y,
                                 float* dw, float* dbias, evt_wgrad_parts* sp, void* stream);
+
+#define EVT_WGRAD_GROUP_MAX 16
+typedef struct evt_wgrad_member {
+  const evt_conv1d_params* p;
+  const void* x;
+  const void* dy;
+  const void* y;
+  float* dw;
+  float* dbias;
+  evt_wgrad_parts* sp;
+} evt_wgrad_member;
+int evt_conv1d_bwd_weight_group(const evt_wgrad_member* members, int32_t n, void* stream);
+
+typedef struct evt_wgrad_plan {
+  int64_t tiles;
+  int32_t stages;
+  int32_t min_stages;
+  int32_t parts;
+  int32_t launch;
+  int32_t nsplit;
+  int32_t per;
+} evt_wgrad_plan;
+int evt_wgrad_group_plan(evt_wgrad_plan* members, int32_t n, int64_t target);
 
 typedef struct evt_resunit_params {
   int32_t dtype, nseq, L, C, k, dil;
```

After: 3541 audio-s/s, median of 6. +1.5%, better.
